# ServiceFoundation/partisan

Hardware: AMD Instinct MI355X
Metric: simulated node-rounds/sec (+ msgs/sec), 1M-node HyParView+Plumtree (higher is better)
Workload: dtype u32

## Files before the change

### partisan_amd/csrc/psim_engine.hip

```cpp
#include <hip/hip_runtime.h>
#include <rccl/rccl.h>

#include <algorithm>
#include <chrono>
#include <cstdio>
#include <cstdlib>
#include <cstring>
#include <new>
#include <set>
#include <vector>

#include "psim_comm.h"
#include "psim_device.h"
#include "psim_kernels.h"
#include "psim_wave.h"

using namespace psim;

namespace {

constexpr int BLK = 256;
constexpr uint32_t PREP_BLK = 1024;
#ifndef PSIM_PREP_NPT
#define PSIM_PREP_NPT 4
// ... 430 lines not shown
            nr++;
        });
    if (nr > FILL_REG) s_spill = 1;
    __syncthreads();
    const bool spill = s_spill != 0;
    bool over = false;
    for (uint32_t j = threadIdx.x; j < nb; j += blockDim.x) {
        const uint32_t c = hcnt[j];
        const uint32_t b0 = c ? atomicAdd(&gcnt[j], c) : 0u;
        over |= b0 + c > capb;
        hcnt[j] = j * capb + b0;
    }
    if (over) ctl[2] = 1;
    __syncthreads();
    const uint32_t wmask = (1u << wshift) - 1;
    auto put = [&](uint32_t g, uint32_t d, uint32_t cls) {
        const uint32_t j = d >> wshift, q = atomicAdd(&hcnt[j], 1u);
        if (q < (j + 1) * capb) pairs[q] = make_uint2((d & wmask) | (cls << 16), g);
    };
    if (!spill) {
#pragma unroll
        for (uint32_t k = 0; k < FILL_REG; k++)
            if (k < nr) put(rg[k], rk[k] & KEY_DST_MASK, rk[k] >> KEY_DST_BITS);
    } else {
        for (uint32_t step = blockIdx.x; step < nsteps; step += gridDim.x) route_step<DENSE>(in, step, spre, sbase, put);
    }
}

template <bool WRITE>
__global__ void __launch_bounds__(RB_STEP) k_owner_part(RouteIn in, uint32_t nsteps, uint32_t spb, uint32_t G,
                                                        uint32_t per, uint32_t* hist,
                                                        const uint32_t* __restrict__ off, Wire* __restrict__ out,
                                                        unsigned long long* mark, uint32_t capH, uint32_t capT,
                                                        const uint32_t* ctl, StatsIn st) {
    if (*ctl) return;
    if (mark && blockIdx.x == 0 && threadIdx.x == 0) *mark = __builtin_amdgcn_s_memrealtime();
    __shared__ uint32_t spre[RB_WAVES][65];
    __shared__ uint64_t sbase[RB_WAVES][64];
    if (!WRITE && blockIdx.x < st.nt) stats_tile(st, blockIdx.x, sbase);
    __shared__ uint32_t wc[RB_WAVES][64], wl[RB_WAVES][64];
    __shared__ uint32_t run[64], runl[64];
    __shared__ uint32_t tb[64];
    const uint32_t w = threadIdx.x >> 6, l = threadIdx.x & 63, nblk = gridDim.x;
    if (threadIdx.x < 64) {
        const uint32_t o = threadIdx.x;
        const bool q = WRITE && o < G;
        if (capH) {
            const uint32_t xs = XHDR + capH;
            run[o] = q ? o * xs + XHDR + off[o * nblk + blockIdx.x] - off[o * nblk] : 0u;
            runl[o] = q ? G * xs + o * capT + off[(G + o) * nblk + blockIdx.x] - off[(G + o) * nblk] : 0u;
            tb[o] = q ? G * xs + o * capT : 0u;
        } else {
            run[o] = q ? off[o * nblk + blockIdx.x] : 0u;
            runl[o] = q ? off[(G + o) * nblk + blockIdx.x] : 0u;
            tb[o] = q ? off[(G + o) * nblk] : 0u;
        }
    }
    if (!WRITE && blockIdx.x == 0 && threadIdx.x == 0) hist[2 * G * nblk] = 0;
    const uint32_t s_end = min(nsteps, (blockIdx.x + 1) * spb);
    for (uint32_t step = blockIdx.x * spb; step < s_end; step++) {
        const uint32_t i = step * RB_STEP + threadIdx.x;
        const uint32_t c = i < in.n_src ? in.ocnt[i] : 0u;
        uint32_t inc = c;
        for (int o = 1; o < 64; o <<= 1) {
            const uint32_t y = __shfl_up(inc, o);
            if (l >= (uint32_t)o) inc += y;
        }
        __syncthreads();
        spre[w][l + 1] = inc;
        if (l == 0) spre[w][0] = 0;
        sbase[w][l] = i < in.n_src ? in.obase[i] : 0ull;
        const uint32_t T = __shfl(inc, 63);
        __syncthreads();
        const uint32_t* pre = spre[w];
        auto rec_at = [&](uint32_t t, uint64_t& g) -> uint32_t {
            if (t >= T) return 0xFFFFFFFFu;
            uint32_t a = 0, b = 64;
            while (b - a > 1) {
                const uint32_t mid = (a + b) >> 1;
                if (pre[mid] <= t) a = mid; else b = mid;
            }
            g = sbase[w][a] + (t - pre[a]);
            return (in.okey[g] & KEY_DST_MASK) / per;
        };
        uint32_t cnt = 0, cntl = 0;
        for (uint32_t t0 = 0; t0 < T; t0 += 64) {
            uint64_t g = 0;
            const uint32_t o = rec_at(t0 + l, g);
            const bool lg = o != 0xFFFFFFFFu && wire_long(in.rec[g].tt);
            for (uint64_t todo = __ballot(o != 0xFFFFFFFFu); todo;) {
                const uint32_t q = __builtin_amdgcn_readlane(o, __ffsll((long long)todo) - 1);
                const uint64_t m = __ballot(o == q), ml = __ballot(o == q && lg);
                cnt += l == q ? (uint32_t)__popcll(m) : 0u;
                cntl += l == q ? (uint32_t)__popcll(ml) : 0u;
                todo &= ~m;
            }
        }
        wc[w][l] = cnt;
        wl[w][l] = cntl;
        __syncthreads();
        if (WRITE) {
            uint32_t B = 0, BL = 0;
            if (l < G) {
                B = run[l];
                BL = runl[l];
                for (uint32_t v = 0; v < w; v++) { B += wc[v][l]; BL += wl[v][l]; }
            }
            for (uint32_t t0 = 0; t0 < T; t0 += 64) {
                uint64_t g = 0;
                const uint32_t o = rec_at(t0 + l, g);
                uint4 x0 = make_uint4(0, 0, 0, 0), x1 = x0, x2 = x0, x3 = x0;
                if (o != 0xFFFFFFFFu) {
                    const uint4* sp = reinterpret_cast<const uint4*>(&in.rec[g]);
                    x0 = sp[0]; x1 = sp[1]; x2 = sp[2]; x3 = sp[3];
                }
                const bool lg = o != 0xFFFFFFFFu && wire_long(x0.z);
                uint32_t pos = 0, lpos = 0;
                for (uint64_t todo = __ballot(o != 0xFFFFFFFFu); todo;) {
                    const uint32_t q = __builtin_amdgcn_readlane(o, __ffsll((long long)todo) - 1);
                    const uint64_t m = __ballot(o == q), ml = __ballot(o == q && lg);
                    const uint64_t below = (1ull << l) - 1ull;
                    if (o == q) {
                        pos = __builtin_amdgcn_readlane(B, q) + (uint32_t)__popcll(m & below);
                        lpos = __builtin_amdgcn_readlane(BL, q) + (uint32_t)__popcll(ml & below);
                    }
                    B += l == q ? (uint32_t)__popcll(m) : 0u;
                    BL += l == q ? (uint32_t)__popcll(ml) : 0u;
                    todo &= ~m;
                }
                if (o != 0xFFFFFFFFu) {
                    if (lg) {
                        x1.w = lpos - tb[o];
                        if (!capH || x1.w < capT) {
                            out[lpos].q[0] = x2;
                            out[lpos].q[1] = x3;
                        }
                    }
                    if (!capH || pos < (o + 1) * (XHDR + capH)) {
                        out[pos].q[0] = x0;
                        out[pos].q[1] = x1;
                    }
                }
            }
        }
        __syncthreads();
        if (threadIdx.x < G)
            for (uint32_t v = 0; v < RB_WAVES; v++) { run[threadIdx.x] += wc[v][threadIdx.x]; runl[threadIdx.x] += wl[v][threadIdx.x]; }
    }
    if (!WRITE) {
        __syncthreads();
        if (threadIdx.x < G) {
            hist[threadIdx.x * nblk + blockIdx.x] = run[threadIdx.x];
            hist[(G + threadIdx.x) * nblk + blockIdx.x] = runl[threadIdx.x];
        }
    }
}

constexpr uint32_t OO_THREADS = 1024;
__global__ void k_owner_offsets(const uint32_t* hoff, uint32_t nblk, uint32_t G, uint64_t* d_off, uint64_t* cnt,
                                uint64_t* xw, uint32_t capH, uint32_t capT, uint32_t* ctl, uint32_t round,
                                uint32_t rank, Wire* sendbuf, StatsIn st) {
    __shared__ uint32_t smh, smt;
    __shared__ uint64_t ssum[64];
    __shared__ uint64_t sred[OO_THREADS / 64][64];
    const uint32_t q = threadIdx.x;
    const bool dead = *ctl != 0;
    if (capH) {
        const uint32_t xs = XHDR + capH;
        uint32_t mh = 0, mt = 0;
        for (uint32_t o = 0; o < G && !dead; o++) {
            mh = max(mh, hoff[(o + 1) * nblk] - hoff[o * nblk]);
            mt = max(mt, hoff[(G + o + 1) * nblk] - hoff[(G + o) * nblk]);
        }
        const bool over = !dead && (mh > capH || mt > capT);
        {
            const uint32_t c = q & 63, g = q >> 6, ng = OO_THREADS / 64;
            uint64_t v = 0;
            if (c < NST) {
#pragma unroll 4
                for (uint32_t b = g; b < st.nt; b += ng) v += st.tiles[(size_t)b * NST + c];
            }
            sred[g][c] = v;
            __syncthreads();
            if (g == 0) {
                uint64_t u = 0;
                for (uint32_t k = 0; k < ng; k++) u += sred[k][c];
                ssum[c] = u;
            }
        }
        __syncthreads();
        for (uint32_t o = 0; o < G; o++) {
            uint64_t* hw = reinterpret_cast<uint64_t*>(sendbuf + (size_t)o * xs);
            const uint64_t c = dead ? 0ull
                                    : (uint64_t)(hoff[(o + 1) * nblk] - hoff[o * nblk]) |
                                          ((uint64_t)(hoff[(G + o + 1) * nblk] - hoff[(G + o) * nblk]) << 32);
            if (q == 0) { hw[XH_CNT] = c; hw[XH_ABORT] = dead || over ? 1u : 0u; hw[XH_MH] = mh; hw[XH_MT] = mt; }
            if (q < NST) hw[XH_STATS + q] = ssum[q];
            if (q == 1) st.hout[PIN_XCNT + o] = c;
        }
        if (q == 0) {
            st.hout[NST] = st.out[NST];
            st.hout[NST + 1] = st.out[NST + 1];
            if (st.outx_top) st.hout0[PIN_OUTX] = *st.outx_top;
            if (over) { ctl[1] = round; __threadfence(); ctl[0] = 3; }
        }
        return;
    }
    if (q <= 2 * G) d_off[q] = hoff[q * nblk];
    if (cnt && q < G)
        cnt[q] = dead ? 0ull
                      : (uint64_t)(hoff[(q + 1) * nblk] - hoff[q * nblk]) |
                            ((uint64_t)(hoff[(G + q + 1) * nblk] - hoff[(G + q) * nblk]) << 32);
    if (!xw) return;
    if (q == 0) {
        uint32_t mh = 0, mt = 0;
        for (uint32_t o = 0; o < G && !dead; o++) {
            mh = max(mh, hoff[(o + 1) * nblk] - hoff[o * nblk]);
            mt = max(mt, hoff[(G + o + 1) * nblk] - hoff[(G + o) * nblk]);
        }
        xw[1] = mh;
        xw[2] = mt;
        smh = mh; smt = mt;
        if (capH && !dead && (mh > capH || mt > capT)) { ctl[1] = round; __threadfence(); ctl[0] = 3; }
    }
    __syncthreads();
    if (q < 128) xw[3 + q] = q == rank ? smh : q == 64 + rank ? smt : 0u;
}




__device__ __forceinline__ void block_sort_lds(uint32_t* sv, uint32_t* p, uint32_t k) {
    uint32_t P = 1;
    while (P < k) P <<= 1;
    for (uint32_t t = threadIdx.x; t < P; t += blockDim.x) sv[t] = t < k ? p[t] : 0xFFFFFFFFu;
    __syncthreads();
    for (uint32_t kk = 2; kk <= P; kk <<= 1) {
        for (uint32_t jj = kk >> 1; jj > 0; jj >>= 1) {
            for (uint32_t t = threadIdx.x; t < P; t += blockDim.x) {
                const uint32_t u = t ^ jj;
                if (u > t) {
                    const uint32_t a = sv[t], b = sv[u];
                    if ((a > b) == ((t & kk) == 0)) { sv[t] = b; sv[u] = a; }
                }
            }
            __syncthreads();
        }
    }
    for (uint32_t t = threadIdx.x; t < k; t += blockDim.x) p[t] = sv[t];
    __syncthreads();
}

__device__ __forceinline__ void sort_run_block(uint32_t* p, uint32_t k, uint32_t* y, uint32_t* sv) {
    for (uint32_t c0 = 0; c0 < k; c0 += RUN_LDS) block_sort_lds(sv, p + c0, min(RUN_LDS, k - c0));
    uint32_t* x = p;
    for (uint32_t wd = RUN_LDS; wd < k; wd *= 2) {
        for (uint32_t a0 = threadIdx.x * 2 * wd; a0 < k; a0 += blockDim.x * 2 * wd) {
            const uint32_t m0 = min(a0 + wd, k), e0 = min(a0 + 2 * wd, k);
            uint32_t u = a0, v = m0, o = a0;
            while (u < m0 && v < e0) y[o++] = x[u] <= x[v] ? x[u++] : x[v++];
            while (u < m0) y[o++] = x[u++];
            while (v < e0) y[o++] = x[v++];
        }
        __syncthreads();
        uint32_t* z = x; x = y; y = z;
    }
    if (x != p)
        for (uint32_t t = threadIdx.x; t < k; t += blockDim.x) p[t] = x[t];
    __syncthreads();
}

__device__ __forceinline__ void wave_sort64(uint32_t* p, uint32_t k) {
    const uint32_t l = threadIdx.x & 63;
    uint32_t v = l < k ? p[l] : 0xFFFFFFFFu;
#pragma unroll
    for (uint32_t kk = 2; kk <= 64; kk <<= 1) {
#pragma unroll
        for (uint32_t j = kk >> 1; j > 0; j >>= 1) {
            const uint32_t u = (uint32_t)__shfl_xor((int)v, (int)j);
            const bool keep_min = ((l & j) == 0) == ((l & kk) == 0);
            v = keep_min ? min(v, u) : max(v, u);
        }
    }
    if (l < k) p[l] = v;
}

__device__ __forceinline__ uint4 wire_piece(const Wire* __restrict__ heads, const Wire* __restrict__ tails,
                                            uint32_t k, uint32_t p) {
    if (p == 0) return heads[k].q[0];
    const uint32_t tt = heads[k].q[0].z;
    const uint4 h1 = heads[k].q[1];
    const bool lng = wire_long(tt);
    if (p == 1) return make_uint4(h1.x, h1.y, h1.z, lng ? 0u : h1.w);
    return lng ? tails[h1.w].q[p - 2] : make_uint4(0, 0, 0, 0);
}

__device__ __forceinline__ uint4 rec_piece(const Msg* __restrict__ rec, uint32_t k, uint32_t p) {
    const uint4 v = reinterpret_cast<const uint4*>(&rec[k])[p];
    if (!PSIM_SHORT_TAIL) return v;
    const uint32_t tt = (uint32_t)__builtin_amdgcn_update_dpp(0, (int)v.z, 0x00, 0xF, 0xF, false);
    return p < 2 || wire_long(tt) ? v : make_uint4(0, 0, 0, 0);
}

template <bool WIRE>
__global__ void __launch_bounds__(RR_THREADS) k_bucket_route(
    uint32_t n, uint32_t wshift, uint32_t regcap, const uint32_t* __restrict__ base,
    const uint2* __restrict__ pairs, const Msg* __restrict__ rec, const Wire* __restrict__ heads,
    const Wire* __restrict__ tails, uint32_t* rank, unsigned long long* cb,
    unsigned long long* bmask, uint32_t* in_beg, uint32_t* idx, uint32_t* tmp, Msg* __restrict__ inbox, uint64_t* hm,
    uint64_t cap, uint32_t* ctl, const uint32_t* gcnt, uint32_t capb, uint32_t round1, StatsIn st, uint32_t lcap) {
    if (*ctl) return;
    extern __shared__ __attribute__((aligned(16))) uint32_t sm[];
    __shared__ __attribute__((aligned(16))) uint32_t spart[RR_THREADS + 4];
    uint32_t& s_nl = spart[RR_THREADS];
    const uint32_t W = 1u << wshift, wmask = W - 1, b = blockIdx.x;
    uint32_t* cnt = sm;
    uint32_t* bs = sm + W;
    unsigned long long* mk = reinterpret_cast<unsigned long long*>(sm + 2 * W);
    uint32_t* pre = bs;
    uint32_t s0, s1, q0;
    if (gcnt) {
        if (b == 0) stats_final(st, reinterpret_cast<uint64_t(*)[64]>(sm));
        const uint32_t nb = gridDim.x, per_t = (nb + blockDim.x - 1) / blockDim.x;
        const uint32_t t0 = min(nb, threadIdx.x * per_t), t1 = min(nb, t0 + per_t);
        uint32_t v = 0;
        for (uint32_t j = t0; j < t1; j++) v += gcnt[j];
        uint32_t m;
        const uint32_t run = block_excl<uint32_t, RR_THREADS>(v, &m);
        if (b >= t0 && b < t1) {
            uint32_t x = run;
            for (uint32_t j = t0; j < b; j++) x += gcnt[j];
            spart[RR_THREADS + 1] = x;
        }
        __syncthreads();
        s0 = spart[RR_THREADS + 1];
        s1 = s0 + gcnt[b];
        q0 = b * capb;
        if (ctl[2] || m > cap) {
            if (b == 0 && threadIdx.x == 0) {
                *(hm + (PIN_OVF - PIN_M)) = max(m, 1u);
                if (round1) { ctl[1] = round1 - 1; __threadfence(); ctl[0] = 2; }
            }
            return;
        }
    } else {
        s0 = base[b]; s1 = base[b + 1]; q0 = s0;
        if (base[gridDim.x] > cap) return;
    }
    pairs += q0;
    rank += q0;
    uint32_t* const ix = lcap && s1 - s0 <= lcap ? sm + 4 * W : idx + s0;
    for (uint32_t j = threadIdx.x; j < 4 * W; j += blockDim.x) sm[j] = 0;
    if (threadIdx.x == 0) s_nl = 0;
    __syncthreads();
    auto count = [&](const uint2& x) {
        const uint32_t dl = x.x & wmask, cls = x.x >> 16;
        const uint32_t r = atomicAdd(&cnt[dl], 1u);
        if (cls == KEY_BCAST) {
            atomicAdd(&bs[dl], 1u);
            const uint32_t a0 = WIRE ? heads[x.y].q[1].x : rec[x.y].a0;
            atomicOr(&mk[dl], 1ull << (a0 % PSIM_MSG_SLOTS));
        } else if (cls) {
            atomicAdd(&bs[dl], cls);
        }
        return r;
    };
    const uint32_t np = s1 - s0;
    const bool inreg = np <= regcap * blockDim.x;
    uint2 px[RR_REG];
    uint32_t pr[RR_REG];
    if (inreg) {
#pragma unroll
        for (uint32_t k = 0; k < RR_REG; k++) {
            const uint32_t p = threadIdx.x + k * blockDim.x;
            px[k] = p < np ? pairs[p] : make_uint2(0, 0);
        }
#pragma unroll
        for (uint32_t k = 0; k < RR_REG; k++)
            if (threadIdx.x + k * blockDim.x < np) pr[k] = count(px[k]);
    } else {
        for (uint32_t p = threadIdx.x; p < np; p += blockDim.x) rank[p] = count(pairs[p]);
    }
    __syncthreads();
    const uint32_t per = W / RR_THREADS, j0 = threadIdx.x * per;
    uint32_t sum = 0;
    for (uint32_t j = 0; j < per; j++) sum += cnt[j0 + j];
    {
        uint32_t tot;
        spart[threadIdx.x] = block_excl<uint32_t, RR_THREADS>(sum, &tot) + sum;
    }
    for (uint32_t dl = threadIdx.x; dl < W; dl += blockDim.x) {
        const uint32_t d = (b << wshift) + dl;
        if (d >= n) break;
        cb[d] = cnt[dl] | ((unsigned long long)bs[dl] << 32);
        bmask[d] = mk[dl];
    }
    __syncthreads();
    uint32_t run = spart[threadIdx.x] - sum;
    for (uint32_t j = 0; j < per; j++) {
        pre[j0 + j] = run;
        run += cnt[j0 + j];
    }
    __syncthreads();
    for (uint32_t dl = threadIdx.x; dl < W; dl += blockDim.x) {
        const uint32_t d = (b << wshift) + dl;
        if (d >= n) break;
        in_beg[d] = s0 + pre[dl];
    }
    if (b == gridDim.x - 1 && threadIdx.x == 0) {
        in_beg[n] = s1;
        *hm = s1;
        if (s1 > hm[PIN_MMAX - PIN_M]) hm[PIN_MMAX - PIN_M] = s1;
    }
    if (inreg) {
#pragma unroll
        for (uint32_t k = 0; k < RR_REG; k++)
            if (threadIdx.x + k * blockDim.x < np) ix[pre[px[k].x & wmask] + pr[k]] = px[k].y;
    } else {
        for (uint32_t p = threadIdx.x; p < np; p += blockDim.x) {
            const uint2 x = pairs[p];
            ix[pre[x.x & wmask] + rank[p]] = x.y;
        }
    }
    __syncthreads();
    uint32_t* sv = reinterpret_cast<uint32_t*>(mk);
    uint32_t* ll = sv + RUN_LDS;
    for (uint32_t dl = threadIdx.x; dl < W; dl += blockDim.x) {
        const uint32_t k = cnt[dl];
        if (k < 2) continue;
        if (k > RUN_SHORT) {
            ll[atomicAdd(&s_nl, 1u)] = dl;
            continue;
        }
        uint32_t* q = ix + pre[dl];
        uint32_t v[RUN_SHORT];
#pragma unroll
        for (uint32_t t = 0; t < RUN_SHORT; t++) v[t] = t < k ? q[t] : 0xFFFFFFFFu;
#pragma unroll
        for (uint32_t r = 0; r < RUN_SHORT; r++) {
#pragma unroll
            for (uint32_t t = r & 1; t + 1 < RUN_SHORT; t += 2) {
                const uint32_t lo_ = v[t], hi_ = v[t + 1];
                v[t] = min(lo_, hi_);
                v[t + 1] = max(lo_, hi_);
            }
        }
#pragma unroll
        for (uint32_t t = 0; t < RUN_SHORT; t++)
            if (t < k) q[t] = v[t];
    }
    __syncthreads();
    const uint32_t nl = s_nl, wv = threadIdx.x >> 6, nwv = blockDim.x >> 6;
    for (uint32_t q = wv; q < nl; q += nwv) {
        const uint32_t dl = ll[q], k = cnt[dl];
        if (k <= 64) wave_sort64(ix + pre[dl], k);
    }
    __syncthreads();
    for (uint32_t q = 0; q < nl; q++) {
        const uint32_t dl = ll[q], k = cnt[dl];
        if (k > 64) sort_run_block(ix + pre[dl], k, tmp + s0 + pre[dl], sv);
    }
    __syncthreads();
    const uint32_t m4 = (s1 - s0) * 4, bd = blockDim.x;
    for (uint32_t t = threadIdx.x; t < m4; t += 2 * bd) {
        const uint32_t t2 = t + bd;
        uint4 a, c = make_uint4(0, 0, 0, 0);
        if (WIRE) {
            a = wire_piece(heads, tails, ix[t >> 2], t & 3);
            if (t2 < m4) c = wire_piece(heads, tails, ix[t2 >> 2], t2 & 3);
        } else {
            a = rec_piece(rec, ix[t >> 2], t & 3);
            if (t2 < m4) c = rec_piece(rec, ix[t2 >> 2], t2 & 3);
        }
        reinterpret_cast<uint4*>(&inbox[s0 + (t >> 2)])[t & 3] = a;
        if (t2 < m4) reinterpret_cast<uint4*>(&inbox[s0 + (t2 >> 2)])[t2 & 3] = c;
    }
}

constexpr uint64_t NODE_STATE_BYTES = 416;

__device__ __forceinline__ bool due(uint32_t period, uint32_t r, uint32_t start) {
    return period > 0 && r > start && ((r - start) % period) == 0;
}

#ifdef PSIM_BOUND_TERMS
enum { BT_RESP, BT_TIMER, BT_PUSH, BT_PUSH_NE, BT_NPUSH, BT_LAZY, BT_ON, BT_NL, BT_LC, BT_CRASH, BT_XBOT,
       BT_BUMP, BT_TOTAL, BT_C, BT_QUIET, BT_ROUNDS, BT_N };
__device__ unsigned long long g_bterm[BT_N];
#define BTERM(k, v) (bt[k] += (v))
#else
#define BTERM(k, v) ((void)0)
#endif

__global__ void __launch_bounds__(BLK) k_node_prep(RoundArgs a, const unsigned long long* bmask, uint64_t* packed,
                                                   uint64_t* part, uint32_t* ocnt, unsigned long long* btot,
                                                   uint32_t per, uint64_t* tiles, uint32_t* gcnt, uint32_t ngcnt) {
    if (*a.ctl) return;
    for (uint32_t j = blockIdx.x * blockDim.x + threadIdx.x; j < ngcnt; j += gridDim.x * blockDim.x) gcnt[j] = 0;
    if (gcnt && blockIdx.x == 0 && threadIdx.x == 0) const_cast<uint32_t*>(a.ctl)[2] = 0;
    __shared__ unsigned long long s_up, s_drop, s_b, s_w, s_qp, s_qf;
    if (threadIdx.x == 0) { s_up = 0; s_drop = 0; s_b = 0; s_w = 0; s_qp = 0; s_qf = 0; }
    if (blockIdx.x == 0 && threadIdx.x == 0) {
        a.ktime[0] = ~0ull; a.ktime[1] = 0; *a.n_slow = 0; *a.n_pt = 0;
        if (a.n_shuf) *a.n_shuf = 0;
        if (a.n_lite) { a.n_lite[0] = 0; a.n_lite[1] = 0; a.n_lite[2] = 0; a.n_lite[3] = 0; }
        if (a.n_ptl) { a.n_ptl[0] = 0; a.n_ptl[1] = 0; a.n_ptl[2] = 0; a.n_ptl[3] = 0; }
        if (a.n_stop) *a.n_stop = 0;
    }
    __syncthreads();
    if (a.upart && a.upart_dirty)
        for (uint32_t g = blockIdx.x * blockDim.x + threadIdx.x; g < a.n_nodes; g += gridDim.x * blockDim.x)
            a.upart[g] = (a.flags[g] & F_UP) ? (upart_t)a.part[g] : UPART_DOWN;
    unsigned long long up = 0, drop = 0, bs = 0, ws = 0;
    unsigned long long qp = 0, qf = 0;
#ifdef PSIM_BOUND_TERMS
    unsigned long long bt[BT_N] = {};
#endif
    const uint32_t i0 = blockIdx.x * per, i1 = min(a.n_local, i0 + per);
    struct PrepIn {
        uint8_t f;
        unsigned long long cbi;
        uint32_t st, org;
        unsigned long long bm;
    };
    auto prep_in = [&](uint32_t i) {
        PrepIn q{0, 0ull, 0u, 0u, 0ull};
        if (i < i1) {
            q.f = a.flags[a.lo + i];
            q.cbi = a.in_cb[i];
            q.st = a.start[i];
            q.org = a.pl ? 0u : a.origin[i];
            q.bm = a.pl ? 0ull : bmask[i];
        }
        return q;
    };
    auto node = [&](uint32_t i, const PrepIn& cur) -> uint64_t {
        uint8_t f = cur.f;
        uint64_t b = 0;
        uint32_t w = 0;
        const unsigned long long cbi = cur.cbi;
        uint32_t c = (uint32_t)cbi;
        const uint32_t st_ = cur.st;
        const uint32_t org_ = cur.org;
        const unsigned long long bm_ = cur.bm;
        if (f & F_UP) {
            uint32_t st = st_, r = a.round;
            if (a.pl) {
                const Hdr& x = a.hdr[i];
                bool pending = x.join_contact != PSIM_NONE;
                bool per = due(a.periodic, r, st);
                bool leave = x.pad1[0] != 0;
                if (a.strategy == PSIM_STRATEGY_FULL)
                    b = a.fanout ? (uint64_t)c + a.fanout + 1
                                 : ((uint64_t)c + 2 + (leave ? 1 : 0)) * (a.n_nodes + 1);
                else
                {
                    const uint64_t vn = x.act_n, vg = vn + c + 1;
                    b = (uint64_t)c + (pending ? 1 + 2 * vg : 0) + (per ? 1 + vg : 0) + (leave ? vn : 0) + 1;
                }
                w = c > 0 || (pending && !x.have) || per || leave;
            } else {
                bool origin = org_ != 0;
                const Hdr& x = a.hdr[i];
                const bool promo = a.random_promotion && due(a.promotion_period, r, st);
                b = (cbi >> 32) + (st == r && x.join_contact != PSIM_NONE ? 1u : 0u) + (promo ? 1u : 0u) +
                    (due(a.shuffle_period, r, st) ? 1u : 0u);
                BTERM(BT_RESP, cbi >> 32);
                BTERM(BT_TIMER, b - (cbi >> 32));
                const unsigned long long bm = c ? bm_ : 0ull;
                const uint32_t pushes = (uint32_t)__popcll(bm) + (origin ? 1u : 0u);
                const bool lazy = a.plumtree && due(a.lazy_tick_period, r, st);
                uint32_t lazy_add = 0, push_sum = 0, union_sum = 0;
                if (pushes) {
                    const uint4 r0 = *reinterpret_cast<const uint4*>(a.pt_rt + (size_t)i * RT_WORDS);
                    const uint2 cn = *reinterpret_cast<const uint2*>(a.pt_rt + (size_t)i * RT_WORDS + RT_EN);
                    const uint32_t rts[4] = {r0.x, r0.y, r0.z, r0.w};
                    auto push = [&](uint32_t root) {
                        uint32_t ne = PSIM_PT_MEMBERS_CAP, nl = 0, ne0 = 0;
#pragma unroll
                        for (int k = 0; k < PSIM_PT_ROOTS; k++)
                            if (rts[k] == root) {
                                ne0 = (cn.x >> (8 * k)) & 0xFFu;
                                ne = max(ne, ne0);
                                nl = (cn.y >> (8 * k)) & 0xFFu;
                            }
                        const uint32_t pb = min(2u * PSIM_ACTIVE_CAP, ne + c);
                        push_sum += pb;
                        lazy_add += nl + c;
                        union_sum += min(pb + nl + c, max((uint32_t)PSIM_PT_MEMBERS_CAP, ne0 + nl) + c);
                        BTERM(BT_PUSH, min(2u * PSIM_ACTIVE_CAP, ne + c));
                        BTERM(BT_PUSH_NE, min(2u * PSIM_ACTIVE_CAP, ne));
                        BTERM(BT_NPUSH, 1);
                        BTERM(BT_NL, nl);
                        BTERM(BT_LC, c);
                    };
                    for (unsigned long long m = bm; m; m &= m - 1) push(a.slots[PSIM_MSG_SLOTS + __ffsll(m) - 1]);
                    if (origin) push((a.lo + i) | PSIM_MAP_BIT);
                }
                if (lazy) {
                    const uint32_t fo = (uint32_t)f >> F_OUTN_SHIFT;
                    const uint32_t on = fo < 15 ? fo : (uint32_t)x.out_n;
                    const uint32_t pl = min(push_sum + min((uint32_t)PSIM_PT_OUT_CAP, on + lazy_add), on + union_sum);
                    b += pl;
                    BTERM(BT_LAZY, pl - push_sum);
                    BTERM(BT_ON, on);
                } else {
                    b += push_sum;
                }
                if (pushes) BTERM(BT_C, c);
                bool exits = false;
                if (a.crash_round) {
                    const uint4* ar = reinterpret_cast<const uint4*>(a.act + (size_t)i * PSIM_ACTIVE_CAP);
                    const uint4 a0 = ar[0], a1 = ar[1];
                    const uint32_t av[8] = {a0.x, a0.y, a0.z, a0.w, a1.x, a1.y, a1.z, a1.w};
                    uint32_t cv[PSIM_CONN_CAP] = {};
                    const uint32_t cn = x.conn_n;
                    if (cn) {
                        const uint4* cr = reinterpret_cast<const uint4*>(a.conn + (size_t)i * PSIM_CONN_CAP);
                        const uint4 c0 = cr[0], c1 = cr[1];
                        cv[0] = c0.x; cv[1] = c0.y; cv[2] = c0.z; cv[3] = c0.w;
                        cv[4] = c1.x; cv[5] = c1.y; cv[6] = c1.z; cv[7] = c1.w;
                    }
#pragma unroll
                    for (int k = 0; k < PSIM_ACTIVE_CAP; k++)
                        if ((uint32_t)k < x.act_n && av[k] < a.n_nodes && av[k] != a.lo + i &&
                            crashed_now(a, av[k])) {
                            b++;
                            BTERM(BT_CRASH, 1);
                            bool down = false;
#pragma unroll
                            for (int j = 0; j < PSIM_CONN_CAP; j++) down |= (uint32_t)j < cn && cv[j] == (av[k] | PSIM_CONN_DOWN);
                            exits |= !down;
                        }
#pragma unroll
                    for (int j = 0; j < PSIM_CONN_CAP; j++)
                        exits |= (uint32_t)j < cn && !(cv[j] & PSIM_CONN_DOWN) && crashed_now(a, cv[j] & KEY_DST_MASK);
                }
                const uint32_t fon = (uint32_t)f >> F_OUTN_SHIFT;
                const bool quiet_ok = a.lazy_tick_period == 1 && !a.lazy_wake && !(f & F_LAZY);
                w = c > 0 || st == r || exits || (fon && !quiet_ok) || origin ||
                    (a.random_promotion && (f & F_LOWACT) && due(a.promotion_period, r, st)) ||
                    due(a.shuffle_period, r, st);
                if (a.xbot) {
                    const bool xb = due(a.xbot_period, r, st);
                    const uint32_t cl = x.conn_cl;
                    b += (xb ? 2u : 0u) + cl;
                    BTERM(BT_XBOT, (xb ? 2u : 0u) + cl);
                    w = w || xb || cl;
                }
                if (w && b == 0) { b = 1; BTERM(BT_BUMP, 1); }
                if (!w && fon && lazy) {
                    qp++;
                    qf += fon < 15 ? fon : (uint32_t)x.out_n;
                    BTERM(BT_QUIET, 1);
                    b = 0;
                }
            }
            up++;
        } else {
            drop += c;
        }
        bs += b;
        ws += w;
        BTERM(BT_TOTAL, b);
        return (b << 32) | w;
    };
    PrepIn q[PREP_CHUNK], qn[PREP_CHUNK];
    const uint32_t cstep = PREP_CHUNK * blockDim.x;
#pragma unroll
    for (uint32_t k = 0; k < PREP_CHUNK; k++) q[k] = prep_in(i0 + threadIdx.x + k * blockDim.x);
    for (uint32_t c0 = i0 + threadIdx.x; c0 < i1; c0 += cstep) {
        uint64_t pk[PREP_CHUNK];
#pragma unroll
        for (uint32_t k = 0; k < PREP_CHUNK; k++) {
            const uint32_t i = c0 + k * blockDim.x;
            pk[k] = i < i1 ? node(i, q[k]) : 0ull;
        }
#pragma unroll
        for (uint32_t k = 0; k < PREP_CHUNK; k++) qn[k] = prep_in(c0 + cstep + k * blockDim.x);
#pragma unroll
        for (uint32_t k = 0; k < PREP_CHUNK; k++) {
            const uint32_t i = c0 + k * blockDim.x;
            if (i < i1) {
                packed[i] = pk[k];
                ocnt[i] = 0;
            }
        }
#pragma unroll
        for (uint32_t k = 0; k < PREP_CHUNK; k++) q[k] = qn[k];
    }
#ifdef PSIM_BOUND_TERMS
    if (blockIdx.x == 0 && threadIdx.x == 0) bt[BT_ROUNDS] = 1;
    for (int k = 0; k < BT_N; k++) {
        unsigned long long v = bt[k];
        for (int o = 32; o > 0; o >>= 1) v += __shfl_xor(v, o);
        if ((threadIdx.x & 63) == 0 && v) atomicAdd(&g_bterm[k], v);
    }
#endif
    for (int o = 32; o > 0; o >>= 1) {
        up += __shfl_xor(up, o);
        drop += __shfl_xor(drop, o);
        bs += __shfl_xor(bs, o);
        ws += __shfl_xor(ws, o);
        qp += __shfl_xor(qp, o);
        qf += __shfl_xor(qf, o);
    }
    if ((threadIdx.x & 63) == 0) {
        if (up) atomicAdd(&s_up, up);
        if (drop) atomicAdd(&s_drop, drop);
        if (bs) atomicAdd(&s_b, bs);
        if (ws) atomicAdd(&s_w, ws);
        if (qp) atomicAdd(&s_qp, qp);
        if (qf) atomicAdd(&s_qf, qf);
    }
    __syncthreads();
    if (threadIdx.x == 0) {
        tiles[blockIdx.x] = (s_b << 32) + s_w;
        if (blockIdx.x == gridDim.x - 1) tiles[gridDim.x] = 0;
    }
    if (threadIdx.x == 0) btot[blockIdx.x] = s_b;
    if (threadIdx.x < NST) {
        uint64_t v = threadIdx.x == ST_UP ? s_up : threadIdx.x == ST_DROPPED ? s_drop : threadIdx.x == ST_PROC ? s_qp
                   : threadIdx.x == ST_FAIL ? s_qf : threadIdx.x == ST_BYTES && !a.pl ? s_w * (2 * NODE_STATE_BYTES)
                   : 0ull;
        part[(size_t)blockIdx.x * NST + threadIdx.x] = v;
    }
}

struct DescIn {
    uint32_t in_beg, cnt, start, origin;
};
__device__ __forceinline__ DescIn desc_in(const RoundArgs& a, uint32_t li, uint64_t pk,
                                          const uint32_t* __restrict__ in_beg,
                                          const unsigned long long* __restrict__ cb,
                                          const uint32_t* __restrict__ start) {
    DescIn d{0, 0, 0, 0};
    if (pk & 1u) {
        d.in_beg = in_beg[li];
        d.cnt = (uint32_t)cb[li];
        d.start = start[li];
        d.origin = a.plumtree && !a.pl ? a.origin[li] : 0u;
    }
    return d;
}

__device__ __forceinline__ void desc_entry(const RoundArgs& a, uint32_t li, uint64_t P, uint64_t pk, const DescIn& d,
                                           uint4* __restrict__ desc, uint64_t* __restrict__ obase, uint32_t* nact,
                                           unsigned long long tot, uint64_t* hout, uint64_t cap, uint32_t* ctl) {
    obase[li] = P >> 32;
    if (li == a.n_local) {
        *nact = (uint32_t)P;
        obase[li] = tot;
        hout[PIN_TOTAL] = tot;
        if (tot > hout[PIN_TMAX]) hout[PIN_TMAX] = tot;
        if (cap && tot + 1 > cap) { ctl[1] = a.round; __threadfence(); ctl[0] = 1; }
        return;
    }
    if (!(pk & 1u)) return;
    if (d.cnt > DESC_CNT_MASK) hout[PIN_BIGIN] = 1;
    const uint32_t st = d.start, r = a.round;
    const uint32_t tf = (a.random_promotion && due(a.promotion_period, r, st) ? DESC_PROMO : 0u) |
                        (due(a.shuffle_period, r, st) ? DESC_SHUFFLE : 0u) |
                        (a.plumtree && due(a.lazy_tick_period, r, st) ? DESC_LAZY : 0u) |
                        (d.origin ? DESC_ORIGIN : 0u);
    const uint32_t xb = a.xbot && due(a.xbot_period, r, st) ? DESC_XBOT_BIT : 0u;
    desc[(uint32_t)P] = make_uint4(a.lo + li, d.in_beg, d.cnt | xb | (tf << 28), (uint32_t)(P >> 32));
}

__device__ unsigned long long btot_sum(const unsigned long long* btot, uint32_t nbt) {
    __shared__ unsigned long long s_w[PREP_BLK / 64], s_tot;
    unsigned long long t = 0;
    for (uint32_t j = threadIdx.x; j < nbt; j += blockDim.x) t += btot[j];
    for (int o = 32; o > 0; o >>= 1) t += __shfl_xor(t, o);
    if ((threadIdx.x & 63) == 0) s_w[threadIdx.x >> 6] = t;
    __syncthreads();
    if (threadIdx.x == 0) {
        unsigned long long u = 0;
        for (uint32_t k = 0; k < blockDim.x / 64; k++) u += s_w[k];
        s_tot = u;
    }
    __syncthreads();
    return s_tot;
}


__global__ void __launch_bounds__(PREP_BLK) k_desc(const uint64_t* __restrict__ packed,
                                                  const uint64_t* __restrict__ tiles, uint32_t per,
                                                  const uint32_t* __restrict__ in_beg,
                                                  const unsigned long long* __restrict__ cb,
                                                  const uint32_t* __restrict__ start, RoundArgs a,
                                                  uint4* __restrict__ desc, uint64_t* __restrict__ obase,
                                                  uint32_t* nact, const unsigned long long* btot,
                                                  uint32_t nranges, uint64_t* hout, uint64_t cap, uint32_t* ctl) {
    if (*ctl) return;
    const bool last = blockIdx.x == gridDim.x - 1;
    const uint32_t r0 = blockIdx.x * DESC_RANGES;
    const uint32_t i0 = r0 * per, i1 = min(a.n_local, i0 + DESC_RANGES * per);
    uint64_t tp = 0;
#pragma unroll
    for (uint32_t k = 0; k < DESC_RANGES; k++) {
        const uint32_t j = threadIdx.x + k * PREP_BLK;
        tp += j < r0 ? tiles[j] : 0ull;
    }
    uint32_t li = i0 + threadIdx.x;
    uint64_t pk = li < i1 ? packed[li] : 0ull;
    DescIn d = desc_in(a, li, pk, in_beg, cb, start);
    const unsigned long long tot = last ? btot_sum(btot, nranges) : 0ull;
    uint64_t carry;
    (void)block_excl<uint64_t, PREP_BLK>(tp, &carry);
    for (uint32_t k = i0; k < i1; k += PREP_BLK) {
        if (k != i0) {
            li = k + threadIdx.x;
            pk = li < i1 ? packed[li] : 0ull;
            d = desc_in(a, li, pk, in_beg, cb, start);
        }
        uint64_t pass;
        const uint64_t e = block_excl<uint64_t, PREP_BLK>(pk, &pass);
        if (li < i1) desc_entry(a, li, carry + e, pk, d, desc, obase, nact, 0ull, hout, cap, ctl);
        carry += pass;
    }
    if (last && threadIdx.x == 0)
        desc_entry(a, a.n_local, carry, 0ull, DescIn{0, 0, 0, 0}, desc, obase, nact, tot, hout, cap, ctl);
}

enum { H_AIN = 0, H_PIN = 1, H_AOUT = 2, H_PFILL = 3, H_HOP = 4, H_NUP = 5 * PSIM_HIST_BINS,
       H_DELIV, H_LAST, H_LINKS, H_N };

__device__ __forceinline__ uint32_t hbin(uint32_t v) { return v < PSIM_HIST_BINS ? v : PSIM_HIST_BINS - 1; }

__global__ void k_hist_out(const Hdr* __restrict__ hdr, const uint32_t* __restrict__ act,
                           const uint32_t* __restrict__ pas, const uint8_t* __restrict__ flags, uint32_t lo,
                           uint32_t n, uint64_t tbit, uint32_t* indeg_a, uint32_t* indeg_p,
                           unsigned long long* hist) {
    __shared__ unsigned long long sh[H_N];
    for (uint32_t j = threadIdx.x; j < H_N; j += blockDim.x) sh[j] = 0;
    __syncthreads();
    const uint32_t i = blockIdx.x * blockDim.x + threadIdx.x;
    if (i < n && (flags[lo + i] & F_UP)) {
        const Hdr& x = hdr[i];
        const uint32_t me = lo + i;
        uint32_t out = 0;
        for (uint32_t k = 0; k < x.act_n; k++) {
            const uint32_t p = act[(size_t)i * PSIM_ACTIVE_CAP + k];
            if (p == me) continue;
            out++;
            if (flags[p] & F_UP) { atomicAdd(&indeg_a[p], 1u); atomicAdd(&sh[H_LINKS], 1ull); }
        }
        for (uint32_t k = 0; k < x.pas_n; k++) {
            const uint32_t p = pas[(size_t)i * PSIM_PASSIVE_CAP + k];
            if (p != me && (flags[p] & F_UP)) atomicAdd(&indeg_p[p], 1u);
        }
        atomicAdd(&sh[H_AOUT * PSIM_HIST_BINS + hbin(out)], 1ull);
        atomicAdd(&sh[H_PFILL * PSIM_HIST_BINS + hbin(x.pas_n)], 1ull);
        atomicAdd(&sh[H_NUP], 1ull);
        if (tbit && ((((uint64_t)x.aux << 32) | x.have) & tbit)) {
            atomicAdd(&sh[H_DELIV], 1ull);
            atomicAdd(&sh[H_HOP * PSIM_HIST_BINS + hbin(x.trk_hop)], 1ull);
            if (x.trk_round != PSIM_NONE) atomicMax(&sh[H_LAST], (unsigned long long)x.trk_round);
        }
    }
    __syncthreads();
    for (uint32_t j = threadIdx.x; j < H_N; j += blockDim.x) {
        if (!sh[j]) continue;
        if (j == H_LAST) atomicMax(&hist[j], sh[j]);
        else atomicAdd(&hist[j], sh[j]);
    }
}

__global__ void k_hist_in(const uint32_t* __restrict__ indeg_a, const uint32_t* __restrict__ indeg_p,
                          const uint8_t* __restrict__ flags, uint32_t lo, uint32_t n, unsigned long long* hist) {
    __shared__ unsigned long long sh[2 * PSIM_HIST_BINS];
    for (uint32_t j = threadIdx.x; j < 2 * PSIM_HIST_BINS; j += blockDim.x) sh[j] = 0;
    __syncthreads();
    const uint32_t i = blockIdx.x * blockDim.x + threadIdx.x;
    if (i < n && (flags[lo + i] & F_UP)) {
        atomicAdd(&sh[hbin(indeg_a[lo + i])], 1ull);
        atomicAdd(&sh[PSIM_HIST_BINS + hbin(indeg_p[lo + i])], 1ull);
    }
    __syncthreads();
    for (uint32_t j = threadIdx.x; j < 2 * PSIM_HIST_BINS; j += blockDim.x)
        if (sh[j]) atomicAdd(&hist[H_AIN * PSIM_HIST_BINS + j], sh[j]);
}

__global__ void k_pack_act(const Hdr* __restrict__ hdr, const uint32_t* __restrict__ act, uint32_t n,
                           uint32_t* gact, uint8_t* gan) {
    const uint32_t i = blockIdx.x * blockDim.x + threadIdx.x;
    if (i >= n) return;
    const uint32_t k = hdr[i].act_n;
    gan[i] = (uint8_t)k;
    for (uint32_t j = 0; j < PSIM_ACTIVE_CAP; j++) gact[(size_t)i * PSIM_ACTIVE_CAP + j] = act[(size_t)i * PSIM_ACTIVE_CAP + j];
}

__global__ void k_hist_sym(const uint8_t* __restrict__ gan, const uint32_t* __restrict__ act,
                           const uint8_t* __restrict__ flags, uint32_t n, unsigned long long* sym) {
    const uint32_t i = blockIdx.x * blockDim.x + threadIdx.x;
    if (i >= n || !(flags[i] & F_UP)) return;
    uint32_t c = 0;
    for (uint32_t k = 0; k < gan[i]; k++) {
        const uint32_t p = act[(size_t)i * PSIM_ACTIVE_CAP + k];
        if (p == i || p >= n || !(flags[p] & F_UP)) continue;
        for (uint32_t q = 0; q < gan[p]; q++)
            if (act[(size_t)p * PSIM_ACTIVE_CAP + q] == i) { c++; break; }
    }
    if (c) atomicAdd(sym, (unsigned long long)c);
}

__global__ void k_cc_init(const uint8_t* __restrict__ flags, uint32_t n, uint32_t* L) {
    const uint32_t i = blockIdx.x * blockDim.x + threadIdx.x;
    if (i < n) L[i] = (flags[i] & F_UP) ? i : PSIM_NONE;
}

__global__ void k_cc_hook(const uint32_t* __restrict__ off, const uint8_t* __restrict__ gan,
                          const uint32_t* __restrict__ act, const uint8_t* __restrict__ flags, uint32_t n,
                          uint32_t* L, uint32_t* changed) {
    const uint32_t i = blockIdx.x * blockDim.x + threadIdx.x;
    if (i >= n || !(flags[i] & F_UP)) return;
    const uint32_t* row = act + (off ? (size_t)off[i] : (size_t)i * PSIM_ACTIVE_CAP);
    for (uint32_t k = 0; k < gan[i]; k++) {
        const uint32_t p = row[k];
        if (p == i || p >= n || !(flags[p] & F_UP)) continue;
        const uint32_t a = L[i], b = L[p];
        if (a < b) { if (atomicMin(&L[p], a) > a) *changed = 1; }
        else if (b < a) { if (atomicMin(&L[i], b) > b) *changed = 1; }
    }
}

__global__ void k_cc_jump(uint32_t n, uint32_t* L) {
    const uint32_t i = blockIdx.x * blockDim.x + threadIdx.x;
    if (i >= n || L[i] == PSIM_NONE) return;
    uint32_t r = L[i];
    while (L[r] != r) r = L[r];
    L[i] = r;
}

__global__ void k_cc_count(const uint32_t* __restrict__ L, uint32_t n, uint32_t* size, unsigned long long* comps) {
    const uint32_t i = blockIdx.x * blockDim.x + threadIdx.x;
    if (i >= n || L[i] == PSIM_NONE) return;
    atomicAdd(&size[L[i]], 1u);
    if (L[i] == i) atomicAdd(comps, 1ull);
}

__global__ void k_cc_max(const uint32_t* __restrict__ size, uint32_t n, unsigned long long* largest) {
    const uint32_t i = blockIdx.x * blockDim.x + threadIdx.x;
    if (i < n && size[i]) atomicMax(largest, (unsigned long long)size[i]);
}

enum { SL_VFILL = 0, SL_IFILL = 1, SL_OUT = 2, SL_NUP = 3 * PSIM_HIST_BINS, SL_VSUM, SL_ISUM, SL_DANG, SL_SELF,
       SL_DUP, SL_IVL, SL_IVC, SL_VMAX, SL_N };
enum { SG_LINKS = PSIM_HIST_BINS, SG_MUTUAL, SG_INMAX, SG_ISOL, SG_COMPS, SG_LARGEST, SG_N };
enum { SF_NUP = 0, SF_MIN, SF_MAX, SF_SUM, SF_AGREE, SF_N };
constexpr uint32_t SH_NPB = BLK;

DEV void sh_row_load(const uint32_t* __restrict__ row, uint32_t n, uint32_t& a, uint32_t& b) {
    const uint32_t l = lane_id();
    a = l < n ? row[l] : PSIM_NONE;
    b = n > 64 && 64 + l < n ? row[64 + l] : PSIM_NONE;
}
DEV void sh_row_first(uint32_t a, uint32_t b, uint32_t n, bool& fa, bool& fb) {
    const uint32_t l = lane_id();
    fa = l < n; fb = 64 + l < n;
    for (uint32_t j = 0; j + 1 < n; j++) {
        const uint32_t v = j < 64 ? shfl(a, (int)j) : shfl(b, (int)(j - 64));
        if (l > j && a == v) fa = false;
        if (64 + l > j && b == v) fb = false;
    }
}
DEV uint32_t sh_wave_sum(uint32_t v) {
    for (int d = 32; d; d >>= 1) v += (uint32_t)__shfl_xor((int)v, d);
    return v;
}
DEV bool sh_live(const uint8_t* __restrict__ flags, uint32_t N, uint32_t id) {
    return id < N && (flags[id] & F_UP);
}

__global__ void __launch_bounds__(BLK) k_sh_rows(const Hdr* __restrict__ hdr, const uint32_t* __restrict__ sview,
                                                 const uint8_t* __restrict__ flags, uint32_t lo, uint32_t n,
                                                 uint32_t N, uint32_t v2, uint8_t* cnt,
                                                 const uint32_t* __restrict__ off, uint32_t* adj,
                                                 unsigned long long* sl) {
    __shared__ unsigned long long sh[SL_N];
    for (uint32_t j = threadIdx.x; j < SL_N; j += blockDim.x) sh[j] = 0;
    __syncthreads();
    const uint32_t l = lane_id();
    const uint32_t base = blockIdx.x * SH_NPB + (threadIdx.x >> 6) * 64;
    const uint32_t mine = base + l;
    uint32_t vn = 0, in_n = 0, o = 0, my_cnt = 0;
    if (mine < n && (flags[lo + mine] & F_UP)) {
        vn = min((uint32_t)hdr[mine].act_n, (uint32_t)PSIM_SVIEW_CAP);
        in_n = hdr[mine].pas_n;
        if (off) o = off[lo + mine];
    }
    const uint64_t up = ballot(mine < n && (flags[lo + mine] & F_UP));
    uint64_t todo = off ? ballot(vn != 0) : up;
    unsigned long long s_vsum = 0, s_isum = 0, s_dang = 0, s_self = 0, s_dup = 0, s_vmax = 0;
    while (todo) {
        const int k = ffs64(todo);
        todo &= todo - 1;
        const uint32_t i = base + (uint32_t)k, me = lo + i;
        const uint32_t len = shfl(vn, k);
        uint32_t a, b;
        bool fa, fb;
        sh_row_load(sview + (size_t)i * PSIM_SVIEW_CAP, len, a, b);
        sh_row_first(a, b, len, fa, fb);
        const uint64_t oa = ballot(fa && a != me), ob = ballot(fb && b != me);
        const uint64_t la = ballot(fa && a != me && sh_live(flags, N, a));
        const uint64_t lb = ballot(fb && b != me && sh_live(flags, N, b));
        if (off) {
            const uint32_t at = shfl(o, k);
            if ((la >> l) & 1) adj[at + popc(la & lt_mask())] = a;
            if ((lb >> l) & 1) adj[at + popc(la) + popc(lb & lt_mask())] = b;
            continue;
        }
        const uint32_t links = popc(la) + popc(lb), others = popc(oa) + popc(ob);
        const uint32_t distinct = popc(ballot(fa)) + popc(ballot(fb));
        if (l == (uint32_t)k) my_cnt = links;
        s_vsum += len; s_dang += others - links; s_self += distinct - others; s_dup += len - distinct;
        s_vmax = len > s_vmax ? len : s_vmax;
        const uint32_t inn = v2 ? shfl(in_n, k) : 0;
        s_isum += inn;
        if (l == 0) {
            atomicAdd(&sh[SL_VFILL * PSIM_HIST_BINS + hbin(len)], 1ull);
            atomicAdd(&sh[SL_OUT * PSIM_HIST_BINS + hbin(others)], 1ull);
            if (v2) atomicAdd(&sh[SL_IFILL * PSIM_HIST_BINS + hbin(inn)], 1ull);
        }
    }
    if (off) return;
    if (mine < n) cnt[lo + mine] = (uint8_t)my_cnt;
    if (l == 0) {
        atomicAdd(&sh[SL_NUP], (unsigned long long)popc(up));
        atomicAdd(&sh[SL_VSUM], s_vsum); atomicAdd(&sh[SL_ISUM], s_isum); atomicAdd(&sh[SL_DANG], s_dang);
        atomicAdd(&sh[SL_SELF], s_self); atomicAdd(&sh[SL_DUP], s_dup); atomicMax(&sh[SL_VMAX], s_vmax);
    }
    __syncthreads();
    for (uint32_t j = threadIdx.x; j < SL_N; j += blockDim.x) {
        if (!sh[j]) continue;
        if (j == SL_VMAX) atomicMax(&sl[j], sh[j]);
        else atomicAdd(&sl[j], sh[j]);
    }
}

DEV bool sh_has(const uint32_t* __restrict__ off, const uint8_t* __restrict__ cnt, const uint32_t* __restrict__ adj,
                uint32_t p, uint32_t id) {
    const uint32_t* row = adj + off[p];
    for (uint32_t q = 0, c = cnt[p]; q < c; q++)
        if (row[q] == id) return true;
    return false;
}

__global__ void __launch_bounds__(BLK) k_sh_inv(const Hdr* __restrict__ hdr, const uint32_t* __restrict__ sinv,
                                                const uint8_t* __restrict__ flags, uint32_t lo, uint32_t n,
                                                uint32_t N, const uint32_t* __restrict__ off,
                                                const uint8_t* __restrict__ cnt, const uint32_t* __restrict__ adj,
                                                unsigned long long* sl) {
    const uint32_t l = lane_id();
    const uint32_t base = blockIdx.x * SH_NPB + (threadIdx.x >> 6) * 64;
    const uint32_t mine = base + l;
    uint32_t in_n = 0;
    if (mine < n && (flags[lo + mine] & F_UP)) in_n = min((uint32_t)hdr[mine].pas_n, (uint32_t)PSIM_SVIEW_CAP);
    uint64_t todo = ballot(in_n != 0);
    uint32_t ivl = 0, ivc = 0;
    while (todo) {
        const int k = ffs64(todo);
        todo &= todo - 1;
        const uint32_t i = base + (uint32_t)k, me = lo + i;
        const uint32_t len = shfl(in_n, k);
        uint32_t a, b;
        bool fa, fb;
        sh_row_load(sinv + (size_t)i * PSIM_SVIEW_CAP, len, a, b);
        sh_row_first(a, b, len, fa, fb);
        if (fa && a != me && sh_live(flags, N, a)) { ivl++; ivc += sh_has(off, cnt, adj, a, me) ? 1u : 0u; }
        if (fb && b != me && sh_live(flags, N, b)) { ivl++; ivc += sh_has(off, cnt, adj, b, me) ? 1u : 0u; }
    }
    ivl = sh_wave_sum(ivl); ivc = sh_wave_sum(ivc);
    if (l == 0 && ivl) atomicAdd(&sl[SL_IVL], (unsigned long long)ivl);
    if (l == 0 && ivc) atomicAdd(&sl[SL_IVC], (unsigned long long)ivc);
}

__global__ void k_sh_rank_tot(const uint32_t* __restrict__ E, uint32_t per, uint32_t W, uint32_t npad,
                              uint32_t* base, unsigned long long* tot) {
    if (blockIdx.x || threadIdx.x) return;
    unsigned long long mx = 0;
    for (uint32_t r = 0; r < W; r++) {
        const uint32_t b = E[min(npad, r * per)], e = E[min(npad, (r + 1) * per)];
        base[r] = b;
        mx = max(mx, (unsigned long long)(e - b));
    }
    tot[0] = mx;
}
__global__ void k_sh_shift(uint32_t* E, uint32_t npad, uint32_t per, uint32_t slot,
                           const uint32_t* __restrict__ base) {
    const uint32_t i = blockIdx.x * blockDim.x + threadIdx.x;
    if (i >= npad) return;
    const uint32_t r = i / per;
    E[i] = E[i] - base[r] + r * slot;
}

__global__ void k_sh_links(const uint32_t* __restrict__ off, const uint8_t* __restrict__ cnt,
                           const uint32_t* __restrict__ adj, uint32_t n, uint32_t* indeg, unsigned long long* sg) {
    __shared__ unsigned long long sh[2];
    if (threadIdx.x < 2) sh[threadIdx.x] = 0;
    __syncthreads();
    const uint32_t i = blockIdx.x * blockDim.x + threadIdx.x;
    const uint32_t c = i < n ? cnt[i] : 0;
    if (c) {
        const uint32_t* row = adj + off[i];
        uint32_t m = 0;
        for (uint32_t k = 0; k < c; k++) {
            const uint32_t p = row[k];
            if (p >= n) continue;
            atomicAdd(&indeg[p], 1u);
            m += sh_has(off, cnt, adj, p, i) ? 1u : 0u;
        }
        atomicAdd(&sh[0], (unsigned long long)c);
        if (m) atomicAdd(&sh[1], (unsigned long long)m);
    }
    __syncthreads();
    if (threadIdx.x < 2 && sh[threadIdx.x]) atomicAdd(&sg[SG_LINKS + threadIdx.x], sh[threadIdx.x]);
}

__global__ void k_sh_in(const uint32_t* __restrict__ indeg, const uint8_t* __restrict__ cnt,
                        const uint8_t* __restrict__ flags, uint32_t n, unsigned long long* sg) {
    __shared__ unsigned long long sh[SG_ISOL + 1];
    for (uint32_t j = threadIdx.x; j <= SG_ISOL; j += blockDim.x) sh[j] = 0;
    __syncthreads();
    const uint32_t i = blockIdx.x * blockDim.x + threadIdx.x;
    if (i < n && (flags[i] & F_UP)) {
        const uint32_t d = indeg[i];
        atomicAdd(&sh[hbin(d)], 1ull);
        atomicMax(&sh[SG_INMAX], (unsigned long long)d);
        if (!d && !cnt[i]) atomicAdd(&sh[SG_ISOL], 1ull);
    }
    __syncthreads();
    for (uint32_t j = threadIdx.x; j <= SG_ISOL; j += blockDim.x) {
        if (!sh[j]) continue;
        if (j == SG_INMAX) atomicMax(&sg[j], sh[j]);
        else atomicAdd(&sg[j], sh[j]);
    }
}

__global__ void k_sh_low(const uint8_t* __restrict__ flags, uint32_t lo, uint32_t n, uint32_t* low) {
    const uint32_t i = blockIdx.x * blockDim.x + threadIdx.x;
    if (i < n && (flags[lo + i] & F_UP)) atomicMin(low, i);
}
__global__ void __launch_bounds__(BLK) k_sh_full(const uint32_t* __restrict__ fbits, const uint8_t* __restrict__ flags,
                                                 uint32_t lo, uint32_t n, uint32_t fw, uint32_t tomb,
                                                 const uint32_t* __restrict__ low, unsigned long long* sf) {
    const uint32_t i = blockIdx.x * (BLK / 64) + (threadIdx.x >> 6);
    if (i >= n || !(flags[lo + i] & F_UP)) return;
    const uint32_t* row = fbits + (size_t)i * 2 * fw;
    const uint32_t* ref = fbits + (size_t)*low * 2 * fw;
    uint32_t c = 0;
    bool differs = false;
    for (uint32_t w = lane_id(); w < fw; w += 64) {
        const uint32_t q = tomb ? row[w] & ~row[fw + w] : row[w];
        const uint32_t r = tomb ? ref[w] & ~ref[fw + w] : ref[w];
        c += (uint32_t)__popc(q);
        differs |= q != r;
    }
    c = sh_wave_sum(c);
    const bool agree = ballot(differs) == 0;
    if (lane_id() == 0) {
        atomicAdd(&sf[SF_NUP], 1ull);
        atomicMin(&sf[SF_MIN], (unsigned long long)c);
        atomicMax(&sf[SF_MAX], (unsigned long long)c);
        atomicAdd(&sf[SF_SUM], (unsigned long long)c);
        if (agree) atomicAdd(&sf[SF_AGREE], 1ull);
    }
}

template <typename T>
struct DBuf {
    T* p = nullptr;
    size_t n = 0;
    int ensure(size_t want, int headroom = 0) {
        if (want <= n) return PSIM_OK;
        static const bool trace = getenv("PSIM_TRACE_GROW") != nullptr;
        if (trace && want >= (1u << 20))
            std::fprintf(stderr, "psim: grow %zu -> %zu (want) x %zu B\n", n, want, sizeof(T));
        if (p) (void)hipFree(p);
        p = nullptr; n = 0;
        const size_t goal = want + want / 4 * (size_t)(headroom > 0 ? headroom : 0);
        size_t cap = 1024;
        while (cap < goal) cap <<= 1;
        if (headroom < 0) cap = want;
        if (cap * sizeof(T) > (1ull << 30)) {
            const size_t step = (64ull << 20) / sizeof(T);
            cap = (want + (headroom < 0 ? 0 : want / 8) + step - 1) / step * step;
        }
        if (hipMalloc(&p, cap * sizeof(T)) != hipSuccess) {
            size_t fr = 0, tot = 0;
            (void)hipGetLastError();
            if (hipMemGetInfo(&fr, &tot) == hipSuccess)
                std::fprintf(stderr, "psim: device allocation of %.2f GB failed (%.2f of %.2f GB free)\n",
                             cap * sizeof(T) / 1e9, fr / 1e9, tot / 1e9);
            p = nullptr;
            return PSIM_ENOMEM;
        }
        n = cap;
        return PSIM_OK;
    }
    int ensure_keep(size_t want, size_t keep, hipStream_t st) {
        if (want <= n) return PSIM_OK;
        if (!p || !keep) return ensure(want);
        DBuf<T> nb;
        TRY(nb.ensure(want));
        if (hipMemcpyAsync(nb.p, p, std::min(keep, n) * sizeof(T), hipMemcpyDeviceToDevice, st) != hipSuccess ||
            hipStreamSynchronize(st) != hipSuccess) {
            nb.release();
            return PSIM_EDEVICE;
        }
        release();
        p = nb.p; n = nb.n;
        return PSIM_OK;
    }
    int alloc(size_t want) {
        static const bool trace = getenv("PSIM_TRACE_GROW") != nullptr;
        if (trace && want >= (1u << 20)) std::fprintf(stderr, "psim: alloc %zu x %zu B\n", want, sizeof(T));
        if (hipMalloc(&p, std::max<size_t>(want, 1) * sizeof(T)) != hipSuccess) return PSIM_ENOMEM;
        n = want;
        if (hipMemset(p, 0, std::max<size_t>(want, 1) * sizeof(T)) != hipSuccess) return PSIM_EDEVICE;
        return PSIM_OK;
    }
    int alloc_on(size_t want, hipStream_t st) {
        if (hipMalloc(&p, std::max<size_t>(want, 1) * sizeof(T)) != hipSuccess) return PSIM_ENOMEM;
        n = want;
        if (hipMemsetAsync(p, 0, std::max<size_t>(want, 1) * sizeof(T), st) != hipSuccess) return PSIM_EDEVICE;
        return PSIM_OK;
    }
    void release() { if (p) (void)hipFree(p); p = nullptr; n = 0; }
};

template <typename T>
struct TmpBuf : DBuf<T> {
    TmpBuf() = default;
    TmpBuf(const TmpBuf&) = delete;
    TmpBuf& operator=(const TmpBuf&) = delete;
    ~TmpBuf() { this->release(); }
};

enum Kern { KT_EVENTS, KT_PREPARE, KT_CONSUME, KT_SCAN, KT_COMPACT, KT_SORT, KT_EXCHANGE, KT_GATHER,
            KT_STATS, KT_N };
const char* kKernName[KT_N] = {"events", "prepare", "consume", "scan", "compact", "sort",
                               "exchange", "gather", "stats"};

inline uint32_t grid_for(uint64_t n) { return (uint32_t)std::max<uint64_t>(1, (n + BLK - 1) / BLK); }

int bits_for(uint64_t n) {
    int b = 1;
    while (b < 32 && (1ull << b) < n) b++;
    return b;
}

constexpr uint64_t RESERVE_PER_NODE = 24;
constexpr uint64_t RCAP_PER_NODE = 4;
constexpr uint64_t RCAP_RESERVE = 8;
constexpr double RCAP_FREE_FRAC = 0.30;
constexpr double OUTBOX_SPARE = 0.12;

struct Shard {
    uint32_t idx = 0, lo = 0, n = 0;
    hipStream_t stream = nullptr;
    DBuf<uint8_t> flags, part;
    DBuf<upart_t> upart;
    DBuf<uint8_t> lite_cm;
    DBuf<uint32_t> crash_bits;
    DBuf<uint8_t> btab;
    DBuf<Hdr> hdr;
    DBuf<uint32_t> act, pas, pt_all, pt_com, pt_eag, pt_laz, pt_rt, start;
    DBuf<uint64_t> sentm, recvm, mapx;
    DBuf<uint32_t> mapx_top;
    DBuf<uint32_t> origin;
    DBuf<uint32_t> slots;
    DBuf<uint32_t> bc_roots, bc_msgs;
    DBuf<uint64_t> pt_out, outx;
    DBuf<uint32_t> conn;
    DBuf<uint32_t> outx_top;
    DBuf<uint32_t> ikeys, ivals;
    uint32_t m_in = 0;
    DBuf<Msg> outbox;
    DBuf<Wire> recvh, recvt;
    DBuf<uint32_t> wseg;
    std::vector<uint32_t> wseg_host;
    DBuf<Msg> inbox;
    DBuf<uint32_t> okey, ocnt, in_beg,
        d_nact, n_slow, n_pt, n_shuf, n_lite, n_ptl, rank, tmp, hist, hoff;
    DBuf<uint32_t> rtot, rbase;
    DBuf<uint32_t> gcnt;
    DBuf<unsigned long long> bmask;
    DBuf<uint2> pairs;
    DBuf<unsigned long long> cb;
    DBuf<unsigned long long> btot;
    DBuf<uint4> desc, desc_slow, desc_pt, desc_shuf, desc_lite, desc_ptl;
    DBuf<uint64_t> bound, pscan, obase, stat_part, stat_out, stat_tile, d_off;
    DBuf<uint8_t> cub_tmp;
    DBuf<uint32_t> ev_ids, ev_contacts, stop_ids, n_stop;
    bool tomb_live = false;
    DBuf<Wire> sendbuf;
    DBuf<uint32_t> sview, sinv, fbits, pay[2], pay_top;
    int pay_cur = 0;
    DBuf<uint8_t> faulted;
    DBuf<uint64_t> omit;
    std::vector<uint64_t> soff, scnt, lcnt;
    uint32_t pper = BLK;
    uint32_t pgrid = 0, cgrid = 0, rgrid = 0, tgrid = 0, sgrid = 0, lgrid = 0, qgrid = 0, egrid = 0;
    uint64_t* pin = nullptr;
    uint64_t* pin_dev = nullptr;
    static constexpr int MAXT = 32;
    hipEvent_t ev[MAXT][2];
    int tk[MAXT];
    int tn = 0;
    hipEvent_t wait_ev = nullptr;
    hipStream_t side[2] = {nullptr, nullptr};
    hipEvent_t fork_ev = nullptr, join_ev[2] = {nullptr, nullptr};
    bool ev_live = false;
    bool reserved = false;
    bool upart_valid = false;
    uint64_t rcap = 0;
    DBuf<uint32_t> ctl;
    uint64_t desc_cap = 0;
    uint32_t batch_round1 = 0;
    uint32_t stat_slot = 0;
    bool outx_short = false;
    uint32_t xcap_h = 0, xcap_t = 0;
    uint32_t xbatch = 1;
    uint64_t trace_tmax = 0, trace_mmax = 0;
};

}

struct psim_handle {
    psim_config cfg;
    uint32_t N = 0, G = 1, per = 0;
    int device = 0;
    uint32_t consume_blocks = 1024;
    uint32_t pt_blocks = 1024;
    uint32_t lite_blocks = 1024;
    psim::LiteKernel lite = {};
    uint32_t ptl_blocks = 1024;
    uint64_t round = 0;
    bool failed = false;
    std::vector<Shard*> shards;
    int rank = 0, world = 1;
    bool ranked = false;
    Comm* comm = nullptr;
    DBuf<uint64_t> comm_cnt;
    uint64_t x_records = 0, x_bytes = 0;
    std::vector<uint32_t> pend_crash, pend_join, pend_contact;
    std::vector<uint8_t> pend_join_mark;
    std::vector<uint32_t> pend_lv_a, pend_lv_t;
    std::vector<uint8_t> pend_part;
    bool pend_part_set = false, pend_part_clear = false;
    std::vector<uint32_t> pend_b_root, pend_b_msg;
    uint32_t slot_tab[2 * PSIM_MSG_SLOTS];
    uint32_t tracked_msg = PSIM_NONE;
    bool btab = false;
    uint32_t btab_hash = 0;
    uint32_t fw = 0;
    bool tomb = false;
    std::vector<uint8_t> started;
    std::set<uint64_t> nx_omit_s, nx_omit_r;
    std::vector<uint8_t> nx_faulted;
    size_t nx_nfaulted = 0;
    bool faults_dirty = false;
    uint32_t faults = 0, n_omit_s = 0, n_omit_r = 0;
    double kt_ms[KT_N] = {0};
    uint64_t kt_n[KT_N] = {0};
    bool phase_timers = false;
    uint32_t rb_blocks = RB_BLOCKS;
    uint32_t rr_reg = RR_REG;
    bool route_fused = true;
};

namespace {

inline bool local_route(const psim_handle* h) { return h->G == 1 && !h->ranked; }

constexpr int PTL_EARLY_DEFAULT = 0;
int ptl_early_knob() {
    static const int v = [] {
        const char* e = getenv("PSIM_PTL_EARLY");
        const int x = e && *e ? atoi(e) : -1;
        return x >= 0 && x <= 2 ? x : PTL_EARLY_DEFAULT;
    }();
    return v;
}

RoundArgs make_args(psim_handle* h, Shard* s) {
    RoundArgs a;
    memset(&a, 0, sizeof a);
    const psim_config& c = h->cfg;
    a.n_nodes = h->N; a.round = (uint32_t)h->round; a.seed = c.seed;
    a.lo = s->lo; a.n_local = s->n;
    a.max_active = c.max_active_size; a.min_active = c.min_active_size;
    a.max_passive = c.max_passive_size; a.arwl = c.arwl; a.prwl = c.prwl;
    a.k_active = c.k_active; a.k_passive = c.k_passive;
    a.shuffle_period = c.shuffle_period; a.promotion_period = c.promotion_period;
    a.random_promotion = c.random_promotion; a.plumtree = c.plumtree;
    a.lazy_tick_period = c.lazy_tick_period;
    a.tracked_msg = h->tracked_msg;
    a.origin = s->origin.p;
    a.slots = s->slots.p;
    a.flags = s->flags.p; a.part = s->part.p; a.hdr = s->hdr.p; a.crash_bits = s->crash_bits.p;
    a.upart = s->upart.p;
    a.lite_cm = s->lite_cm.p;
    a.btab = h->btab ? s->btab.p : nullptr;
    a.act = s->act.p; a.pas = s->pas.p; a.sentm = s->sentm.p; a.recvm = s->recvm.p;
    a.mapx = s->mapx.p; a.mapx_top = s->mapx_top.p;
    a.mapx_rows = (uint32_t)(s->mapx.n / IDMAP_EXT);
    a.pt_all = s->pt_all.p; a.pt_com = s->pt_com.p; a.pt_eag = s->pt_eag.p; a.pt_laz = s->pt_laz.p;
    a.pt_rt = s->pt_rt.p;
    a.pt_out = s->pt_out.p; a.outx = s->outx.p; a.outx_top = s->outx_top.p;
    a.conn = s->conn.p;
    a.outx_rows = (uint32_t)(s->outx.n / OUT_EXT);
    a.start = s->start.p;
    a.pl = c.manager == PSIM_MANAGER_PLUGGABLE;
    a.xbot = c.manager == PSIM_MANAGER_XBOT; a.xbot_period = c.xbot_period;
    a.ptl_split = ptl_early_knob() != 0;
    a.strategy = c.strategy; a.periodic = c.periodic_interval; a.scamp_c = c.scamp_c;
    a.fanout = c.fanout; a.fw = h->fw; a.tomb = h->tomb;
    a.fbits = s->fbits.p; a.sview = s->sview.p; a.sinv = s->sinv.p;
    a.ktime = reinterpret_cast<unsigned long long*>(s->stat_out.p + NST);
    a.ctl = s->ctl.p;
    a.desc_slow = s->desc_slow.p; a.n_slow = s->n_slow.p;
    a.desc_pt = s->desc_pt.p; a.n_pt = s->n_pt.p;
    a.desc_shuf = s->desc_shuf.p; a.n_shuf = s->n_shuf.p;
    a.desc_lite = s->desc_lite.p; a.n_lite = s->n_lite.p;
    a.desc_ptl = s->desc_ptl.p; a.n_ptl = s->n_ptl.p;
    a.stop_ids = s->stop_ids.p; a.n_stop = s->n_stop.p;
    a.faults = h->faults; a.n_omit_s = h->n_omit_s; a.n_omit_r = h->n_omit_r;
    a.faulted = s->faulted.p; a.omit = s->omit.p;
    return a;
}

int route_buffers(Shard* s, bool both_inboxes);

struct KTimer {
    Shard* s;
    int slot;
    KTimer(psim_handle* h, Shard* s_, int k) : s(s_), slot(-1) {
        if (!h->phase_timers || s->tn >= Shard::MAXT) return;
        slot = s->tn++;
        s->tk[slot] = k;
        (void)hipEventRecord(s->ev[slot][0], s->stream);
    }
    ~KTimer() {
        if (slot >= 0) (void)hipEventRecord(s->ev[slot][1], s->stream);
    }
};

void flush_timers(psim_handle* h, Shard* s) {
    for (int i = 0; i < s->tn; i++) {
        float ms = 0;
        if (hipEventElapsedTime(&ms, s->ev[i][0], s->ev[i][1]) != hipSuccess) continue;
        h->kt_ms[s->tk[i]] += ms;
        h->kt_n[s->tk[i]]++;
    }
    s->tn = 0;
}

constexpr uint32_t SCAN_ITEMS = 8, SCAN_TILE = BLK * SCAN_ITEMS;

template <typename T, uint32_t NT>
__device__ T block_excl(T v, T* total) {
    __shared__ T wsum[NT / 64];
    const uint32_t l = threadIdx.x & 63, wv = threadIdx.x >> 6;
    T x = v;
#pragma unroll
    for (int d = 1; d < 64; d <<= 1) {
        const T y = __shfl_up(x, d);
        if (l >= (uint32_t)d) x += y;
    }
    if (l == 63) wsum[wv] = x;
    __syncthreads();
    T base = 0, tot = 0;
#pragma unroll
    for (uint32_t k = 0; k < NT / 64; k++) {
        base += k < wv ? wsum[k] : T(0);
        tot += wsum[k];
    }
    __syncthreads();
    *total = tot;
    return base + x - v;
}

template <typename T, typename TI>
__global__ void __launch_bounds__(BLK) k_scan_tiles(const TI* __restrict__ in, uint32_t n, T* __restrict__ sums) {
    const size_t b0 = (size_t)blockIdx.x * SCAN_TILE + (size_t)threadIdx.x * SCAN_ITEMS;
    T v = 0;
#pragma unroll
    for (uint32_t k = 0; k < SCAN_ITEMS; k++) v += b0 + k < n ? in[b0 + k] : T(0);
    T tot;
    (void)block_excl(v, &tot);
    if (threadIdx.x == 0) sums[blockIdx.x] = tot;
}

constexpr uint32_t SUMS_LDS = 4096 + 2 * BLK;
template <typename T>
__global__ void __launch_bounds__(BLK) k_scan_sums(T* sums, uint32_t nt) {
    __shared__ T buf[SUMS_LDS];
    const bool lds = nt <= SUMS_LDS;
    T* p = lds ? buf : sums;
    if (lds) {
        for (uint32_t i = threadIdx.x; i < nt; i += BLK) buf[i] = sums[i];
        __syncthreads();
    }
    const uint32_t per = (nt + BLK - 1) / BLK, i0 = threadIdx.x * per, i1 = min(nt, i0 + per);
    T v = 0;
    for (uint32_t i = i0; i < i1; i++) v += p[i];
    T tot;
    T run = block_excl(v, &tot);
    for (uint32_t i = i0; i < i1; i++) {
        const T x = p[i];
        p[i] = run;
        run += x;
    }
    if (lds) {
        __syncthreads();
        for (uint32_t i = threadIdx.x; i < nt; i += BLK) sums[i] = buf[i];
    }
}

template <typename T, typename TI>
__global__ void __launch_bounds__(BLK) k_scan_apply(const TI* __restrict__ in, T* __restrict__ out, uint32_t n,
                                                   const T* __restrict__ sums) {
    const size_t b0 = (size_t)blockIdx.x * SCAN_TILE + (size_t)threadIdx.x * SCAN_ITEMS;
    T x[SCAN_ITEMS], v = 0;
#pragma unroll
    for (uint32_t k = 0; k < SCAN_ITEMS; k++) {
        x[k] = b0 + k < n ? in[b0 + k] : T(0);
        v += x[k];
    }
    T tot;
    T run = block_excl(v, &tot) + (sums ? sums[blockIdx.x] : T(0));
#pragma unroll
    for (uint32_t k = 0; k < SCAN_ITEMS; k++) {
        if (b0 + k < n) out[b0 + k] = run;
        run += x[k];
    }
}

template <typename T, typename TI>
int scan_excl(Shard* s, const TI* in, T* out, uint32_t n) {
    const uint32_t nt = (uint32_t)(((uint64_t)n + SCAN_TILE - 1) / SCAN_TILE);
    if (nt <= 1) {
        k_scan_apply<T, TI><<<1, BLK, 0, s->stream>>>(in, out, n, nullptr);
    } else {
        TRY(s->cub_tmp.ensure((size_t)nt * sizeof(T)));
        T* sums = reinterpret_cast<T*>(s->cub_tmp.p);
        k_scan_tiles<T, TI><<<nt, BLK, 0, s->stream>>>(in, n, sums);
        k_scan_sums<T><<<1, BLK, 0, s->stream>>>(sums, nt);
        k_scan_apply<T, TI><<<nt, BLK, 0, s->stream>>>(in, out, n, sums);
    }
    HIP_TRY(hipGetLastError());
    return PSIM_OK;
}

int scan_desc(Shard* s, const RoundArgs& a) {
    k_desc<<<(s->pgrid + DESC_RANGES - 1) / DESC_RANGES, PREP_BLK, 0, s->stream>>>(
        s->bound.p, s->pscan.p, s->pper, s->in_beg.p, s->cb.p, s->start.p, a, s->desc.p, s->obase.p, s->d_nact.p,
        s->btot.p, s->pgrid, s->pin_dev, s->desc_cap, s->ctl.p);
    HIP_TRY(hipGetLastError());
    return PSIM_OK;
}

int stream_wait(Shard* s) {
    HIP_TRY(hipEventRecord(s->wait_ev, s->stream));
    hipError_t e;
    while ((e = hipEventQuery(s->wait_ev)) == hipErrorNotReady) {
    }
    if (e != hipSuccess) {
        static bool said = false;
        if (!said) std::fprintf(stderr, "psim: event query: %s; synchronising\n", hipGetErrorString(e));
        said = true;
        HIP_TRY(hipStreamSynchronize(s->stream));
    }
    return PSIM_OK;
}

template <typename T>
T read1(Shard* s, const T* p) {
    T v{};
    (void)hipMemcpyAsync(&v, p, sizeof(T), hipMemcpyDeviceToHost, s->stream);
    (void)stream_wait(s);
    return v;
}

int upload(Shard* s, DBuf<uint32_t>& b, const std::vector<uint32_t>& v) {
    TRY(b.ensure(v.size()));
    HIP_TRY(hipMemcpyAsync(b.p, v.data(), v.size() * 4, hipMemcpyHostToDevice, s->stream));
    return PSIM_OK;
}

struct RoundCtl {
    bool crashes = false;
    uint64_t bcast_clear = 0;
};

int phase_events_prepare(psim_handle* h, Shard* s, const RoundCtl& ctl, RoundArgs& a, bool events = true,
                         bool batched = false, bool redo = false) {
    const uint32_t n = s->n;
    if (events && h->faults_dirty) {
        std::vector<uint64_t> keys(h->nx_omit_s.begin(), h->nx_omit_s.end());
        keys.insert(keys.end(), h->nx_omit_r.begin(), h->nx_omit_r.end());
        TRY(s->faulted.ensure(h->N));
        TRY(s->omit.ensure(std::max<size_t>(keys.size(), 1)));
        HIP_TRY(hipMemcpyAsync(s->faulted.p, h->nx_faulted.data(), h->N, hipMemcpyHostToDevice, s->stream));
        if (!keys.empty())
            HIP_TRY(hipMemcpyAsync(s->omit.p, keys.data(), keys.size() * 8, hipMemcpyHostToDevice, s->stream));
        HIP_TRY(hipStreamSynchronize(s->stream));
    }
    a = make_args(h, s);
    a.crash_round = ctl.crashes;
    a.upart_dirty = !s->upart_valid ||
                    (events && (ctl.crashes || !h->pend_join.empty() || h->pend_part_set || h->pend_part_clear));
    a.lazy_wake = !s->upart_valid || ((events || redo) && (h->pend_part_set || h->pend_part_clear ||
                                                            h->faults_dirty || !h->pend_lv_a.empty()));
    s->upart_valid = true;
    if (events) {
        KTimer t(h, s, KT_EVENTS);
        if (ctl.crashes) {
            TRY(upload(s, s->ev_ids, h->pend_crash));
            k_crash<<<grid_for(h->pend_crash.size()), BLK, 0, s->stream>>>(
                s->flags.p, s->crash_bits.p, s->ev_ids.p, (uint32_t)h->pend_crash.size());
        }
        if (!h->pend_join.empty()) {
            TRY(upload(s, s->ev_ids, h->pend_join));
            TRY(upload(s, s->ev_contacts, h->pend_contact));
            k_join<<<grid_for(h->pend_join.size()), BLK, 0, s->stream>>>(
                a, s->start.p, s->ev_ids.p, s->ev_contacts.p, (uint32_t)h->pend_join.size(),
                h->cfg.persist_epoch);
        }
        if (!h->pend_lv_a.empty()) {
            TRY(upload(s, s->ev_ids, h->pend_lv_a));
            TRY(upload(s, s->ev_contacts, h->pend_lv_t));
            k_leave_set<<<grid_for(h->pend_lv_a.size()), BLK, 0, s->stream>>>(
                s->hdr.p, s->lo, s->n, s->ev_ids.p, s->ev_contacts.p, (uint32_t)h->pend_lv_a.size());
        }
        if (h->pend_part_clear) HIP_TRY(hipMemsetAsync(s->part.p, 0, h->N, s->stream));
        if (h->pend_part_set)
            HIP_TRY(hipMemcpyAsync(s->part.p, h->pend_part.data(), h->N, hipMemcpyHostToDevice, s->stream));
        if (!h->pend_b_root.empty()) {
            const uint32_t k = (uint32_t)h->pend_b_root.size();
            k_bcast_reset<<<grid_for(n), BLK, 0, s->stream>>>(s->hdr.p, n, (uint32_t)ctl.bcast_clear,
                                                               (uint32_t)(ctl.bcast_clear >> 32));
            TRY(upload(s, s->bc_roots, h->pend_b_root));
            TRY(upload(s, s->bc_msgs, h->pend_b_msg));
            HIP_TRY(hipMemcpyAsync(s->slots.p, h->slot_tab, sizeof h->slot_tab, hipMemcpyHostToDevice, s->stream));
            k_origin<<<grid_for(k), BLK, 0, s->stream>>>(s->origin.p, s->lo, n, s->bc_roots.p, s->bc_msgs.p, k,
                                                          s->flags.p, false, s->ctl.p);
        }
    }
    {
        KTimer t(h, s, KT_PREPARE);
        a.in_cb = s->cb.p;
        {
            const uint32_t g = std::min<uint32_t>(std::max<uint32_t>(1, grid_for(n) / PREP_NPT), DESC_RANGES * PREP_BLK);
            s->pper = BLK * (uint32_t)(((uint64_t)n + (uint64_t)g * BLK - 1) / ((uint64_t)g * BLK));
            s->pgrid = std::max<uint32_t>(1, (uint32_t)(((uint64_t)n + s->pper - 1) / s->pper));
        }
        s->cgrid = std::min<uint32_t>(grid_for(n), h->consume_blocks);
        const bool hv = h->cfg.manager != PSIM_MANAGER_PLUGGABLE;
        s->rgrid = hv ? std::min<uint32_t>(grid_for(n), RELAY_MAX_BLOCKS) : 0;
        s->tgrid = hv && h->cfg.plumtree ? std::min<uint32_t>(grid_for(n), h->pt_blocks) : 0;
        s->sgrid = hv ? std::min<uint32_t>(grid_for(n), SHUF_MAX_BLOCKS) : 0;
        const uint32_t lnodes = h->lite.grid_nodes;
        s->lgrid = hv ? std::min<uint32_t>((uint32_t)((n + lnodes - 1) / lnodes), h->lite_blocks) : 0;
        const uint32_t qnodes = PTL_BLOCK;
        s->qgrid = hv && h->cfg.plumtree ? std::min<uint32_t>((uint32_t)((n + qnodes - 1) / qnodes), h->ptl_blocks) : 0;
        s->egrid = ptl_early_knob() ? s->qgrid : 0;
        TRY(s->stat_part.ensure((size_t)(s->pgrid + s->cgrid + s->rgrid + s->tgrid + s->sgrid + s->lgrid + s->qgrid + s->egrid) *
                                NST));
        k_node_prep<<<s->pgrid, BLK, 0, s->stream>>>(a, s->bmask.p, s->bound.p, s->stat_part.p, s->ocnt.p,
                                                     s->btot.p, s->pper, s->pscan.p, s->gcnt.p, (uint32_t)s->gcnt.n);
        TRY(scan_desc(s, a));
        if (batched) goto args;
        TRY(stream_wait(s));
        if (s->pin[PIN_BIGIN]) { s->pin[PIN_BIGIN] = 0; return PSIM_ENOMEM; }
        const uint64_t total = s->pin[PIN_TOTAL];
        if (total >= 0xFFFFFFFFull) return PSIM_ENOMEM;
        uint64_t want = total + 1;
        int headroom = 2;
        const char* rcap_init = getenv("PSIM_RCAP_INIT");
        if (local_route(h) && !s->rcap) {
            s->rcap = 4096;
            while (s->rcap < (uint64_t)n * RCAP_PER_NODE) s->rcap <<= 1;
            if (rcap_init) s->rcap = std::max<uint64_t>(16, strtoull(rcap_init, nullptr, 10));
        }
        if (!s->reserved) {
            s->reserved = true;
            size_t fr = 0, tot = 0;
            if (!getenv("PSIM_NO_RESERVE") && hipMemGetInfo(&fr, &tot) == hipSuccess) {
                const uint64_t per_rec = sizeof(Msg) + 3 * sizeof(uint32_t) + sizeof(uint2);
                const uint64_t per_slot = sizeof(Msg) + sizeof(uint32_t);
                uint64_t avail = fr + (uint64_t)s->outbox.n * sizeof(Msg) + (uint64_t)s->okey.n * 4;
                static const uint64_t res_pn = getenv("PSIM_RESERVE_PER_NODE")
                                                   ? strtoull(getenv("PSIM_RESERVE_PER_NODE"), nullptr, 10) : RESERVE_PER_NODE;
                static const uint64_t rcap_pn = getenv("PSIM_RCAP_RESERVE")
                                                    ? strtoull(getenv("PSIM_RCAP_RESERVE"), nullptr, 10) : RCAP_RESERVE;
                if (local_route(h) && !rcap_init) {
                    const uint64_t rc = (uint64_t)n * rcap_pn;
                    if (rc > s->rcap && (double)(rc * per_rec) <= RCAP_FREE_FRAC * (double)avail) s->rcap = rc;
                    const uint64_t held = s->rcap * per_rec;
                    avail = avail > held ? avail - held : 0;
                }
                const uint64_t r = std::min<uint64_t>((uint64_t)n * res_pn,
                                                      (uint64_t)((1.0 - OUTBOX_SPARE) * (double)avail) / per_slot);
                if (r > want) {
                    want = r;
                    headroom = -1;
                    s->outbox.release();
                    s->okey.release();
                }
            }
        } else if (want > s->outbox.n && s->outbox.n * sizeof(Msg) > (1ull << 30)) {
            std::fprintf(stderr, "psim: round %llu: outbox grows past its reservation (%zu -> %llu slots)\n",
                         (unsigned long long)h->round, s->outbox.n, (unsigned long long)want);
        }
        TRY(s->outbox.ensure(want, headroom));
        TRY(s->okey.ensure(want, headroom));
        if (local_route(h)) TRY(route_buffers(s, s->m_in == 0));
    }
args:
    a.in_beg = s->in_beg.p;
    a.desc = s->desc.p; a.n_alist = s->d_nact.p;
    a.rec_in = s->inbox.p;
    a.obase = s->obase.p;
    a.rec_out = s->outbox.p;
    a.okey = s->okey.p; a.ocnt = s->ocnt.p;
    a.stat_part = s->stat_part.p + (size_t)s->pgrid * NST;
    a.stat_relay = s->stat_part.p + (size_t)(s->pgrid + s->cgrid) * NST;
    a.stat_pt = s->stat_part.p + (size_t)(s->pgrid + s->cgrid + s->rgrid) * NST;
    a.stat_shuf = s->stat_part.p + (size_t)(s->pgrid + s->cgrid + s->rgrid + s->tgrid) * NST;
    a.stat_lite = s->stat_part.p + (size_t)(s->pgrid + s->cgrid + s->rgrid + s->tgrid + s->sgrid) * NST;
    a.stat_ptl = s->stat_part.p + (size_t)(s->pgrid + s->cgrid + s->rgrid + s->tgrid + s->sgrid + s->lgrid) * NST;
    a.stat_ptle = s->egrid ? a.stat_ptl + (size_t)s->qgrid * NST : nullptr;
    return PSIM_OK;
}

constexpr int PHASE_FUSED_DEFAULT = 3;

void launch_lite(psim_handle* h, Shard* s, const RoundArgs& a, hipStream_t st) {
    h->lite.kernel<<<s->lgrid, h->lite.block, 0, st>>>(a);
}

int phase_consume(psim_handle* h, Shard* s, RoundArgs& a) {
    if (a.pl && a.strategy == PSIM_STRATEGY_FULL) {
        uint64_t slots = (uint64_t)s->m_in + s->n + 1;
        if (slots > 0xFFFFFFFFull) return PSIM_ENOMEM;
        TRY(s->pay[s->pay_cur].ensure(slots * 2 * h->fw));
        if (h->tomb && !s->tomb_live) {
            DBuf<uint32_t>& in = s->pay[s->pay_cur ^ 1];
            const size_t rows = in.n / (2 * h->fw);
            if (rows)
                HIP_TRY(hipMemset2DAsync(in.p + h->fw, 2 * h->fw * 4, 0, h->fw * 4, rows, s->stream));
            s->tomb_live = true;
        }
        a.pay_out = s->pay[s->pay_cur].p;
        a.pay_in = s->pay[s->pay_cur ^ 1].p;
        a.pay_top = s->pay_top.p;
        a.pay_cap = (uint32_t)(s->pay[s->pay_cur].n / (2 * h->fw));
        HIP_TRY(hipMemsetAsync(s->pay_top.p, 0, 4, s->stream));
    }
    if (a.pl) {
        k_consume_pl<<<s->cgrid, BLK, 0, s->stream>>>(a);
    } else {
        k_relay<<<s->rgrid, BLK, 0, s->stream>>>(a);
        RoundArgs b = a;
        b.desc = s->desc_slow.p;
        b.n_alist = s->n_slow.p;
        static const bool conc_env = getenv("PSIM_CONCURRENT_PHASE") != nullptr;
        static const bool serial_env = getenv("PSIM_SERIAL_PHASE") != nullptr;
        const bool serial = serial_env || a.crash_round || !(conc_env || h->lite.side_by_side);
        static const int fused_env = [] {
            const char* e = getenv("PSIM_PHASE_FUSED");
            const int v = e && *e ? atoi(e) : PHASE_FUSED_DEFAULT;
            return v == 2 || v == 3 ? v : 0;
        }();
        const bool fused = fused_env && !a.crash_round && !serial_env && !conc_env && h->lite.kernel == k_lite_quarter;
        const int early = fused && fused_env == 3 && s->egrid ? ptl_early_knob() : 0;
        if (fused) {
            const uint32_t lg = fused_env == 3 ? s->lgrid : 0, eg = early == 1 ? s->egrid : 0;
            if (s->sgrid + s->cgrid + lg + eg)
                k_hv_phase<<<s->sgrid + s->cgrid + lg + eg, BLK, 0, s->stream>>>(a, s->sgrid, s->cgrid, eg);
            if (fused_env == 2) launch_lite(h, s, a, s->stream);
        } else if (serial) {
            k_shuf<<<s->sgrid, BLK, 0, s->stream>>>(a);
            launch_lite(h, s, a, s->stream);
            k_consume<<<s->cgrid, BLK, 0, s->stream>>>(b);
        } else {
            HIP_TRY(hipEventRecord(s->fork_ev, s->stream));
            HIP_TRY(hipStreamWaitEvent(s->side[0], s->fork_ev, 0));
            HIP_TRY(hipStreamWaitEvent(s->side[1], s->fork_ev, 0));
            k_consume<<<s->cgrid, BLK, 0, s->side[0]>>>(b);
            k_shuf<<<s->sgrid, BLK, 0, s->side[1]>>>(a);
            launch_lite(h, s, a, s->stream);
            for (int k = 0; k < 2; k++) {
                HIP_TRY(hipEventRecord(s->join_ev[k], s->side[k]));
                HIP_TRY(hipStreamWaitEvent(s->stream, s->join_ev[k], 0));
            }
        }
        if (s->qgrid) {
            if (early == 2) k_ptl_part<<<s->egrid, PTL_BLOCK, 0, s->stream>>>(a, PTL_EARLY);
            if (early) k_ptl_part<<<s->qgrid, PTL_BLOCK, 0, s->stream>>>(a, PTL_LATE);
            else k_ptl<<<s->qgrid, PTL_BLOCK, 0, s->stream>>>(a);
        }
        if (s->tgrid) {
            RoundArgs c = a;
            c.desc = s->desc_pt.p;
            c.n_alist = s->n_pt.p;
            c.stat_part = a.stat_pt;
            k_pt<<<s->tgrid, BLK, 0, s->stream>>>(c);
        }
    }
    HIP_TRY(hipGetLastError());
    s->pay_cur ^= 1;
    return PSIM_OK;
}

unsigned long long* phase_end_mark(psim_handle* h, Shard* s) {
    return h->cfg.manager == PSIM_MANAGER_PLUGGABLE ? nullptr
                                                    : reinterpret_cast<unsigned long long*>(s->stat_out.p + NST) + 1;
}

int route_group(psim_handle* h, Shard* s, bool dense, uint32_t m, bool fixed = false, bool exact = false) {
    const uint32_t n = s->n;
    uint32_t wshift = n > (1u << 26) ? 13 : n > (1u << 22) ? 12 : 11;
    if (const char* e = getenv("PSIM_ROUTE_WSHIFT")) {
        const int v = atoi(e);
        if (v >= (int)WSHIFT_MIN && v <= (int)WSHIFT_MAX) wshift = (uint32_t)v;
    }
    const uint32_t W = 1u << wshift, nb = (n + W - 1) >> wshift;
    const RouteIn in{s->outbox.p, s->okey.p, s->obase.p, s->ocnt.p, dense ? m : n, s->lo,
                     h->cfg.manager == PSIM_MANAGER_PLUGGABLE, dense ? s->recvh.p : nullptr,
                     dense ? s->recvt.p : nullptr, dense && !fixed ? s->wseg.p : nullptr, dense ? h->G : 0u,
                     fixed ? s->xcap_h : 0u, fixed ? s->xcap_t : 0u, (uint32_t)h->round};
    const uint32_t nsteps = std::max<uint32_t>(1, (in.n_src + RB_STEP - 1) / RB_STEP);
    const uint32_t nblk = std::min<uint32_t>(nsteps, h->rb_blocks);
    const size_t nh = (size_t)nb * nblk;
    TRY(s->hist.ensure(nh));
    TRY(s->hoff.ensure(nh));
    TRY(s->rtot.ensure(nb));
    TRY(s->rbase.ensure(nb + 1));
    static const bool lidx_ok = !getenv("PSIM_ROUTE_LIDX") || atoi(getenv("PSIM_ROUTE_LIDX")) != 0;
    const uint32_t lcap = lidx_ok && W == (1u << WSHIFT_MIN) ? ROUTE_LIDX : 0u;
    const size_t lds_h = (size_t)nb * 4, lds_r = (size_t)W * 16 + (size_t)lcap * 4;
    const uint32_t rows = s->pgrid + s->cgrid + s->rgrid + s->tgrid + s->sgrid + s->lgrid + s->qgrid + s->egrid;
    const StatsIn st{s->stat_part.p, rows,
                     fixed ? 0u : std::min<uint32_t>(nblk, std::min<uint32_t>(STAT_TILES, std::max<uint32_t>(1, rows / 32))),
                     s->stat_tile.p, s->stat_out.p, s->pin_dev + (size_t)s->stat_slot * PIN_STRIDE,
                     s->outx.p ? s->outx_top.p : nullptr, s->pin_dev};
    KTimer t(h, s, KT_SORT);
    if (!dense && !exact && h->route_fused && n <= (1u << 26)) {
        const uint64_t capb64 = (s->rcap + nb - 1) / nb * 3 / 2 + 64;
        const uint32_t capb = (uint32_t)std::min<uint64_t>(capb64, 0xFFFFFFFFull / nb);
        if (s->gcnt.n < nb) {
            TRY(s->gcnt.ensure(nb));
            HIP_TRY(hipMemsetAsync(s->gcnt.p, 0, s->gcnt.n * 4, s->stream));
        }
        TRY(s->pairs.ensure((size_t)nb * capb));
        TRY(s->rank.ensure((size_t)nb * capb));
        static const uint32_t walk = getenv("PSIM_FILL_WALK") && atoi(getenv("PSIM_FILL_WALK")) ? 1u : 0u;
        k_bucket_fill<false><<<nblk, RB_STEP, lds_h, s->stream>>>(in, nsteps, nb, wshift, s->gcnt.p, capb, s->pairs.p,
                                                                  s->ctl.p, phase_end_mark(h, s), st, walk);
        k_bucket_route<false><<<nb, RR_THREADS, lds_r, s->stream>>>(
            n, wshift, h->rr_reg, nullptr, s->pairs.p, in.rec, nullptr, nullptr, s->rank.p, s->cb.p, s->bmask.p,
            s->in_beg.p, s->ivals.p, s->tmp.p, s->inbox.p, s->pin_dev + PIN_M, s->rcap, s->ctl.p, s->gcnt.p, capb,
            s->batch_round1, st, lcap);
        HIP_TRY(hipGetLastError());
        return PSIM_OK;
    }
    if (dense)
        k_bucket_hist<true><<<nblk, RB_STEP, lds_h, s->stream>>>(in, nsteps, nb, wshift, s->hist.p, s->ctl.p,
                                                                 nullptr, st);
    else
        k_bucket_hist<false><<<nblk, RB_STEP, lds_h, s->stream>>>(in, nsteps, nb, wshift, s->hist.p, s->ctl.p,
                                                                  phase_end_mark(h, s), st);
    k_bucket_offsets<<<nb, RB_MAX_BLOCKS, 0, s->stream>>>(s->hist.p, nblk, s->hoff.p, s->rtot.p, s->ctl.p);
    if (dense)
        k_bucket_scatter<true><<<nblk, RB_STEP, lds_h, s->stream>>>(in, nsteps, nb, wshift, s->hoff.p, s->rtot.p,
                                                                    s->rbase.p, s->pairs.p, s->rcap,
                                                                    s->pin_dev + PIN_OVF, s->ctl.p,
                                                                    s->batch_round1, st);
    else
        k_bucket_scatter<false><<<nblk, RB_STEP, lds_h, s->stream>>>(in, nsteps, nb, wshift, s->hoff.p, s->rtot.p,
                                                                     s->rbase.p, s->pairs.p, s->rcap,
                                                                     s->pin_dev + PIN_OVF, s->ctl.p,
                                                                     s->batch_round1, st);
    if (dense)
        k_bucket_route<true><<<nb, RR_THREADS, lds_r, s->stream>>>(
            n, wshift, h->rr_reg, s->rbase.p, s->pairs.p, nullptr, in.wire, in.tails, s->rank.p, s->cb.p, s->bmask.p,
            s->in_beg.p, s->ivals.p, s->tmp.p, s->inbox.p, s->pin_dev + PIN_M, s->rcap, s->ctl.p, nullptr, 0u,
            s->batch_round1, st, lcap);
    else
        k_bucket_route<false><<<nb, RR_THREADS, lds_r, s->stream>>>(
            n, wshift, h->rr_reg, s->rbase.p, s->pairs.p, in.rec, nullptr, nullptr, s->rank.p, s->cb.p, s->bmask.p,
            s->in_beg.p, s->ivals.p, s->tmp.p, s->inbox.p, s->pin_dev + PIN_M, s->rcap, s->ctl.p, nullptr, 0u,
            s->batch_round1, st, lcap);
    HIP_TRY(hipGetLastError());
    return PSIM_OK;
}

int route_buffers(Shard* s, bool both_inboxes) {
    const size_t c = s->rcap + 1;
    TRY(s->ivals.ensure(c)); TRY(s->tmp.ensure(c)); TRY(s->rank.ensure(c)); TRY(s->pairs.ensure(c));
    (void)both_inboxes;
    TRY(s->inbox.ensure_keep(c, s->m_in, s->stream));
    return PSIM_OK;
}

int phase_route_local(psim_handle* h, Shard* s, bool exact = false) { return route_group(h, s, false, 0, false, exact); }

void send_counts(Shard* s, uint32_t G);

int phase_partition(psim_handle* h, Shard* s, bool fixed = false) {
    const uint32_t G = h->G;
    RouteIn in{};
    in.rec = s->outbox.p; in.okey = s->okey.p; in.obase = s->obase.p; in.ocnt = s->ocnt.p; in.n_src = s->n;
    const uint32_t nsteps = std::max<uint32_t>(1, (s->n + RB_STEP - 1) / RB_STEP);
    const uint32_t spb = (nsteps + h->rb_blocks - 1) / h->rb_blocks;
    const uint32_t nblk = (nsteps + spb - 1) / spb;
    const size_t nh = (size_t)2 * G * nblk + 1;
    TRY(s->hist.ensure(nh));
    TRY(s->hoff.ensure(nh));
    if (!fixed) TRY(s->sendbuf.ensure(2 * (s->pin[PIN_TOTAL] + 1), 2));
    TRY(s->d_off.ensure(2 * G + 1));
    const bool rccl = h->ranked;
    if (rccl) TRY(h->comm_cnt.ensure(2 * G + 2));
    s->soff.assign(2 * G + 1, 0);
    const uint32_t capH = fixed ? s->xcap_h : 0u, capT = fixed ? s->xcap_t : 0u;
    StatsIn st{};
    if (fixed) {
        const uint32_t rows = s->pgrid + s->cgrid + s->rgrid + s->tgrid + s->sgrid + s->lgrid + s->qgrid + s->egrid;
        st = StatsIn{s->stat_part.p, rows,
                     std::min<uint32_t>(nblk, std::min<uint32_t>(STAT_TILES, std::max<uint32_t>(1, rows / 32))),
                     s->stat_tile.p, s->stat_out.p, s->pin_dev + (size_t)s->stat_slot * PIN_STRIDE,
                     s->outx.p ? s->outx_top.p : nullptr, s->pin_dev};
    }
    {
        KTimer t(h, s, KT_SORT);
        k_owner_part<false><<<nblk, RB_STEP, 0, s->stream>>>(in, nsteps, spb, G, h->per, s->hist.p, nullptr,
                                                              nullptr, phase_end_mark(h, s), capH, capT, s->ctl.p, st);
        TRY(scan_excl(s, s->hist.p, s->hoff.p, (uint32_t)nh));
        k_owner_part<true><<<nblk, RB_STEP, 0, s->stream>>>(in, nsteps, spb, G, h->per, nullptr, s->hoff.p,
                                                             s->sendbuf.p, nullptr, capH, capT, s->ctl.p, StatsIn{});
        k_owner_offsets<<<1, OO_THREADS, 0, s->stream>>>(s->hoff.p, nblk, G, s->d_off.p, rccl ? h->comm_cnt.p : nullptr,
                                                  rccl ? s->stat_out.p + STAT_OUT_X : nullptr, capH, capT, s->ctl.p,
                                                  (uint32_t)h->round, s->idx, s->sendbuf.p, st);
        HIP_TRY(hipGetLastError());
        if (rccl) return PSIM_OK;
        HIP_TRY(hipMemcpyAsync(s->soff.data(), s->d_off.p, (2 * G + 1) * 8, hipMemcpyDeviceToHost, s->stream));
        TRY(stream_wait(s));
    }
    send_counts(s, G);
    return PSIM_OK;
}

void send_counts(Shard* s, uint32_t G) {
    s->scnt.resize(G);
    s->lcnt.resize(G);
    for (uint32_t g = 0; g < G; g++) {
        s->scnt[g] = s->soff[g + 1] - s->soff[g];
        s->lcnt[g] = s->soff[G + g + 1] - s->soff[G + g];
    }
}

int phase_receive(psim_handle* h, Shard* s, const std::vector<uint64_t>& hc, const std::vector<uint64_t>& lc) {
    const uint32_t G = h->G;
    s->wseg_host.assign(2 * (G + 1), 0);
    uint64_t m = 0, ml = 0;
    for (uint32_t g = 0; g < G; g++) {
        s->wseg_host[g] = (uint32_t)m;
        s->wseg_host[G + 1 + g] = (uint32_t)ml;
        m += hc[g];
        ml += lc[g];
    }
    s->wseg_host[G] = (uint32_t)m;
    s->wseg_host[2 * G + 1] = (uint32_t)ml;
    TRY(s->wseg.ensure(2 * (G + 1)));
    HIP_TRY(hipMemcpyAsync(s->wseg.p, s->wseg_host.data(), s->wseg_host.size() * 4, hipMemcpyHostToDevice,
                           s->stream));
    s->rcap = std::max<uint64_t>(s->rcap, m);
    TRY(route_buffers(s, false));
    TRY(route_group(h, s, true, (uint32_t)m));
    s->m_in = (uint32_t)m;
    return PSIM_OK;
}

int exchange_local(psim_handle* h) {
    const uint32_t G = h->G;
    for (Shard* d : h->shards) {
        std::vector<uint64_t> hc(G), lc(G);
        uint64_t m = 0, ml = 0;
        for (Shard* s : h->shards) {
            hc[s->idx] = s->scnt[d->idx];
            lc[s->idx] = s->lcnt[d->idx];
            m += hc[s->idx];
            ml += lc[s->idx];
        }
        TRY(d->recvh.ensure(m + 1));
        TRY(d->recvt.ensure(ml + 1));
        {
            KTimer t(h, d, KT_EXCHANGE);
            uint64_t oh = 0, ot = 0;
            for (uint32_t g = 0; g < G; g++) {
                Shard* s = h->shards[g];
                if (hc[g])
                    HIP_TRY(hipMemcpyAsync(d->recvh.p + oh, s->sendbuf.p + s->soff[d->idx], hc[g] * sizeof(Wire),
                                           hipMemcpyDeviceToDevice, d->stream));
                if (lc[g])
                    HIP_TRY(hipMemcpyAsync(d->recvt.p + ot, s->sendbuf.p + s->soff[G + d->idx], lc[g] * sizeof(Wire),
                                           hipMemcpyDeviceToDevice, d->stream));
                if (g != d->idx) {
                    h->x_records += hc[g];
                    h->x_bytes += (hc[g] + lc[g]) * sizeof(Wire);
                }
                oh += hc[g];
                ot += lc[g];
            }
        }
        TRY(phase_receive(h, d, hc, lc));
    }
    return PSIM_OK;
}

int exchange_rccl(psim_handle* h) {
    Shard* s = h->shards[0];
    const uint32_t G = h->G;
    std::vector<uint64_t> hc(G), lc(G);
    {
        KTimer t(h, s, KT_EXCHANGE);
        TRY(h->comm->all_to_all_u64(h->comm_cnt.p, h->comm_cnt.p + G, 1, s->stream));
        std::vector<uint64_t> rcnt(G);
        HIP_TRY(hipMemcpyAsync(rcnt.data(), h->comm_cnt.p + G, G * 8, hipMemcpyDeviceToHost, s->stream));
        HIP_TRY(hipMemcpyAsync(s->soff.data(), s->d_off.p, (2 * G + 1) * 8, hipMemcpyDeviceToHost, s->stream));
        TRY(stream_wait(s));
        send_counts(s, G);
        uint64_t m = 0, ml = 0;
        std::vector<uint64_t> roh(G), rot(G);
        for (uint32_t g = 0; g < G; g++) {
            hc[g] = rcnt[g] & 0xFFFFFFFFull;
            lc[g] = rcnt[g] >> 32;
            roh[g] = m;
            rot[g] = ml;
            m += hc[g];
            ml += lc[g];
        }
        TRY(s->recvh.ensure(m + 1));
        TRY(s->recvt.ensure(ml + 1));
        std::vector<Xfer> sends, recvs;
        const bool self_comm = h->world == 1;
        for (uint32_t g = 0; g < G; g++) {
            if (g == s->idx && !self_comm) continue;
            if (s->scnt[g]) sends.push_back({(int)g, s->sendbuf.p + s->soff[g], s->scnt[g] * sizeof(Wire)});
            if (s->lcnt[g]) sends.push_back({(int)g, s->sendbuf.p + s->soff[G + g], s->lcnt[g] * sizeof(Wire)});
            if (hc[g]) recvs.push_back({(int)g, s->recvh.p + roh[g], hc[g] * sizeof(Wire)});
            if (lc[g]) recvs.push_back({(int)g, s->recvt.p + rot[g], lc[g] * sizeof(Wire)});
            h->x_records += s->scnt[g];
            h->x_bytes += (s->scnt[g] + s->lcnt[g]) * sizeof(Wire);
        }
        TRY(h->comm->exchange(sends, recvs, s->stream));
        if (!self_comm) {
            const uint32_t g = s->idx;
            if (hc[g])
                HIP_TRY(hipMemcpyAsync(s->recvh.p + roh[g], s->sendbuf.p + s->soff[g], hc[g] * sizeof(Wire),
                                       hipMemcpyDeviceToDevice, s->stream));
            if (lc[g])
                HIP_TRY(hipMemcpyAsync(s->recvt.p + rot[g], s->sendbuf.p + s->soff[G + g], lc[g] * sizeof(Wire),
                                       hipMemcpyDeviceToDevice, s->stream));
        }
    }
    return phase_receive(h, s, hc, lc);
}

int exchange_fixed(psim_handle* h) {
    Shard* s = h->shards[0];
    const uint32_t G = h->G, capT = s->xcap_t;
    const size_t xs = XHDR + s->xcap_h;
    KTimer t(h, s, KT_EXCHANGE);
    std::vector<Xfer> sends, recvs;
    const bool self_comm = h->world == 1;
    for (uint32_t g = 0; g < G; g++) {
        if (g == s->idx && !self_comm) continue;
        sends.push_back({(int)g, s->sendbuf.p + g * xs, xs * sizeof(Wire)});
        sends.push_back({(int)g, s->sendbuf.p + G * xs + (size_t)g * capT, (size_t)capT * sizeof(Wire)});
        recvs.push_back({(int)g, s->recvh.p + g * xs, xs * sizeof(Wire)});
        recvs.push_back({(int)g, s->recvt.p + (size_t)g * capT, (size_t)capT * sizeof(Wire)});
    }
    TRY(h->comm->exchange(sends, recvs, s->stream));
    if (!self_comm) {
        const uint32_t g = s->idx;
        HIP_TRY(hipMemcpyAsync(s->recvh.p + g * xs, s->sendbuf.p + g * xs, xs * sizeof(Wire), hipMemcpyDeviceToDevice,
                               s->stream));
        HIP_TRY(hipMemcpyAsync(s->recvt.p + (size_t)g * capT, s->sendbuf.p + G * xs + (size_t)g * capT,
                               (size_t)capT * sizeof(Wire), hipMemcpyDeviceToDevice, s->stream));
    }
    return route_group(h, s, true, (uint32_t)(G * xs), true);
}

void xcaps_set(Shard* s, uint64_t mh, uint64_t mt, bool grow = false, bool shrink = true) {
    const uint64_t ch = std::min<uint64_t>(grow ? 2 * mh + 1024 : mh + mh / 2 + 1024, 0x7FFFFFFFull);
    const uint64_t ct = std::min<uint64_t>(grow ? 2 * mt + 1024 : mt + mt / 2 + 1024, 0x7FFFFFFFull);
    if (ch > s->xcap_h || (shrink && 2 * mh < s->xcap_h)) s->xcap_h = (uint32_t)ch;
    if (ct > s->xcap_t || (shrink && 2 * mt < s->xcap_t)) s->xcap_t = (uint32_t)ct;
}
void xcaps_max(psim_handle* h, const uint64_t* p, uint64_t& mh, uint64_t& mt) {
    for (int r = 0; r < h->world && r < 64; r++) {
        mh = std::max<uint64_t>(mh, p[PIN_XRANK + r]);
        mt = std::max<uint64_t>(mt, p[PIN_XRANK + 64 + r]);
    }
}
void xcaps_update(psim_handle* h, Shard* s, const uint64_t* p) {
    uint64_t mh = 0, mt = 0;
    xcaps_max(h, p, mh, mt);
    xcaps_set(s, mh, mt, false, false);
}

int phase_stats(psim_handle* h, Shard* s, const std::vector<uint32_t>& crashed, bool batched = false) {
    KTimer t(h, s, KT_STATS);
    if (h->ranked && !batched) {
        uint64_t* pw = s->pin_dev + (size_t)s->stat_slot * PIN_STRIDE;
        TRY(h->comm->all_reduce(s->stat_out.p, STAT_OUT_N, CType::U64, COp::SUM, s->stream));
        HIP_TRY(hipMemcpyAsync(pw, s->stat_out.p, NST * 8, hipMemcpyDeviceToDevice, s->stream));
        HIP_TRY(hipMemcpyAsync(pw + PIN_XRANK, s->stat_out.p + STAT_OUT_R, 128 * 8, hipMemcpyDeviceToDevice, s->stream));
    }
    if (!crashed.empty()) {
        TRY(upload(s, s->ev_ids, crashed));
        k_uncrash<<<grid_for(crashed.size()), BLK, 0, s->stream>>>(s->flags.p, s->crash_bits.p, s->ev_ids.p,
                                                                  (uint32_t)crashed.size(), s->ctl.p);
    }
    return PSIM_OK;
}

void bcast_slots(psim_handle* h, RoundCtl& ctl) {
    if (!h->pend_b_root.empty()) {
        for (size_t i = 0; i < h->pend_b_root.size(); i++) {
            const uint32_t k = h->pend_b_msg[i] % PSIM_MSG_SLOTS;
            ctl.bcast_clear |= 1ull << k;
            h->slot_tab[k] = h->pend_b_msg[i];
            h->slot_tab[PSIM_MSG_SLOTS + k] = h->pend_b_root[i] | PSIM_MAP_BIT;
        }
        h->tracked_msg = h->pend_b_msg.back();
    }
}

int run_round(psim_handle* h, uint64_t* st, bool events_applied = false, bool from_partition = false) {
    RoundCtl ctl;
    ctl.crashes = !h->pend_crash.empty();
    if (!events_applied) bcast_slots(h, ctl);
    if (h->faults_dirty) {
        if (h->nx_faulted.size() != h->N) h->nx_faulted.assign(h->N, 0);
        h->n_omit_s = (uint32_t)h->nx_omit_s.size();
        h->n_omit_r = (uint32_t)h->nx_omit_r.size();
        h->faults = h->n_omit_s || h->n_omit_r || h->nx_nfaulted;
    }
    for (Shard* s : h->shards) s->tn = 0;
    std::vector<RoundArgs> args(h->shards.size());
    for (size_t i = 0; i < h->shards.size() && !from_partition; i++)
        TRY(phase_events_prepare(h, h->shards[i], ctl, args[i], !events_applied, false, events_applied));
    static const long long fail_round = getenv("PSIM_TEST_FAIL_ROUND") ? atoll(getenv("PSIM_TEST_FAIL_ROUND")) : -1;
    if (fail_round >= 0 && h->round == (uint64_t)fail_round) {
        for (Shard* s : h->shards) (void)hipStreamSynchronize(s->stream);
        return PSIM_ENOMEM;
    }
    for (size_t i = 0; i < h->shards.size() && !from_partition; i++) TRY(phase_consume(h, h->shards[i], args[i]));
    if (local_route(h)) {
        TRY(phase_route_local(h, h->shards[0]));
    } else {
        for (Shard* s : h->shards) TRY(phase_partition(h, s));
        if (h->ranked) TRY(exchange_rccl(h));
        else TRY(exchange_local(h));
    }
    for (Shard* s : h->shards) {
        TRY(phase_stats(h, s, h->pend_crash));
        if (!h->pend_b_root.empty())
            k_origin<<<grid_for(h->pend_b_root.size()), BLK, 0, s->stream>>>(
                s->origin.p, s->lo, s->n, s->bc_roots.p, s->bc_msgs.p, (uint32_t)h->pend_b_root.size(), s->flags.p,
                true, s->ctl.p);
    }
    memset(st, 0, NST * 8);
    for (Shard* s : h->shards) {
        TRY(stream_wait(s));
        flush_timers(h, s);
        for (int k = 0; k < NST; k++) st[k] += s->pin[k];
        if (local_route(h) && s->pin[PIN_OVF]) {
            const uint64_t m = s->pin[PIN_OVF];
            s->pin[PIN_OVF] = 0;
            if (s->rcap < m + m / 2) {
                const uint64_t want = m + m / 2;
                if (want <= (1ull << 26)) while (s->rcap < want) s->rcap <<= 1;
                else s->rcap = (want + (1ull << 20) - 1) >> 20 << 20;
            }
            TRY(route_buffers(s, false));
            TRY(phase_route_local(h, s, true));
            TRY(stream_wait(s));
        }
        if (local_route(h)) s->m_in = (uint32_t)s->pin[PIN_M];
        if (h->ranked) xcaps_update(h, s, s->pin);
        static const bool trace_relay = getenv("PSIM_TRACE_RELAY") != nullptr;
        if (trace_relay && s->rgrid)
        {
            uint64_t em = 0;
            for (int k = 0; k < ST_NTYPES; k++) em += s->pin[ST_EMIT + k];
            std::fprintf(stderr, "psim: round %llu shard %u: %u nodes with work, %u to k_consume, %u to k_pt, "
                         "%u to k_shuf, %u to k_consume_lite, %u to k_ptl, outbox bound %llu, emitted %llu\n",
                         (unsigned long long)h->round, s->idx, read1(s, s->d_nact.p), read1(s, s->n_slow.p),
                         read1(s, s->n_pt.p), read1(s, s->n_shuf.p), read1(s, s->n_lite.p) + read1(s, s->n_lite.p + 1) + read1(s, s->n_lite.p + 2) + read1(s, s->n_lite.p + 3),
                         read1(s, s->n_ptl.p) + read1(s, s->n_ptl.p + 1) + read1(s, s->n_ptl.p + 2) + read1(s, s->n_ptl.p + 3),
                         (unsigned long long)s->pin[PIN_TOTAL], (unsigned long long)em);
        }
        if (s->pin[NST] != ~0ull && s->pin[NST + 1] > s->pin[NST]) {
            h->kt_ms[KT_CONSUME] += (double)(s->pin[NST + 1] - s->pin[NST]) * 1e-5;
            h->kt_n[KT_CONSUME]++;
        }
    }
    if (st[ST_BOUND]) {
        std::fprintf(stderr, "psim: round %llu: %llu nodes emitted past their outbox bound (engine bug)\n",
                     (unsigned long long)h->round, (unsigned long long)st[ST_BOUND]);
        return PSIM_EDEVICE;
    }
    for (uint32_t j : h->pend_join) h->pend_join_mark[j] = 0;
    h->pend_crash.clear(); h->pend_join.clear(); h->pend_contact.clear();
    h->pend_lv_a.clear(); h->pend_lv_t.clear();
    if (st[ST_STOP]) {
        std::vector<uint32_t> ids;
        for (Shard* s : h->shards) {
            const size_t k = read1(s, s->n_stop.p);
            if (!k) continue;
            const size_t at = ids.size();
            ids.resize(at + k);
            HIP_TRY(hipMemcpyAsync(ids.data() + at, s->stop_ids.p, k * 4, hipMemcpyDeviceToHost, s->stream));
            TRY(stream_wait(s));
        }
        if (h->ranked) {
            Shard* s = h->shards[0];
            const uint32_t W = h->world;
            std::vector<uint64_t> cnt(W), mine(ids.begin(), ids.end());
            const uint64_t k = mine.size();
            TRY(h->comm_cnt.ensure(W + 1));
            HIP_TRY(hipMemcpyAsync(h->comm_cnt.p + W, &k, 8, hipMemcpyHostToDevice, s->stream));
            TRY(h->comm->all_gather(h->comm_cnt.p + W, h->comm_cnt.p, 8, s->stream));
            HIP_TRY(hipMemcpyAsync(cnt.data(), h->comm_cnt.p, W * 8, hipMemcpyDeviceToHost, s->stream));
            TRY(stream_wait(s));
            const uint64_t mk = *std::max_element(cnt.begin(), cnt.end());
            mine.resize(mk, 0);
            std::vector<uint64_t> all((size_t)W * mk);
            TRY(h->comm_cnt.ensure((size_t)W * mk + mk));
            HIP_TRY(hipMemcpyAsync(h->comm_cnt.p + (size_t)W * mk, mine.data(), mk * 8, hipMemcpyHostToDevice,
                                   s->stream));
            TRY(h->comm->all_gather(h->comm_cnt.p + (size_t)W * mk, h->comm_cnt.p, mk * 8, s->stream));
            HIP_TRY(hipMemcpyAsync(all.data(), h->comm_cnt.p, all.size() * 8, hipMemcpyDeviceToHost, s->stream));
            TRY(stream_wait(s));
            ids.clear();
            for (uint32_t r = 0; r < W; r++)
                for (uint64_t j = 0; j < cnt[r]; j++) ids.push_back((uint32_t)all[(size_t)r * mk + j]);
        }
        std::sort(ids.begin(), ids.end());
        h->pend_crash.insert(h->pend_crash.end(), ids.begin(), ids.end());
    }
    h->pend_part_set = h->pend_part_clear = false;
    h->faults_dirty = false;
    h->pend_b_root.clear(); h->pend_b_msg.clear();
    h->round++;
    return PSIM_OK;
}

void fill_stats(const uint64_t* s, uint64_t round, psim_round_stats* o) {
    memset(o, 0, sizeof *o);
    o->round = round;
    for (int i = 0; i < ST_NTYPES; i++) {
        o->emitted[i] = s[ST_EMIT + i];
        o->delivered[i] = s[ST_DELIV + i];
    }
    o->dropped = s[ST_DROPPED]; o->nodes_up = s[ST_UP]; o->nodes_processed = s[ST_PROC];
    o->exits = s[ST_EXITS]; o->send_fail = s[ST_FAIL]; o->first_deliveries = s[ST_FIRST];
    o->overflow = s[ST_OVF]; o->digest = s[ST_DIGEST]; o->state_bytes = s[ST_BYTES];
    for (int k = 0; k < PSIM_OVF_NKINDS; k++) o->overflow_by[k] = s[ST_OVF_BY + k];
    o->omitted = s[ST_OMIT];
}

bool batchable(psim_handle* h) {
    static const bool trace = getenv("PSIM_TRACE_RELAY") != nullptr;
    static const bool off = getenv("PSIM_NO_BATCH") != nullptr || getenv("PSIM_TEST_FAIL_ROUND") != nullptr;
    static const bool off_ranked = getenv("PSIM_NO_RANK_BATCH") != nullptr;
    if (off || trace || h->phase_timers || h->cfg.strict || h->cfg.manager == PSIM_MANAGER_PLUGGABLE ||
        !h->pend_lv_a.empty())
        return false;
    Shard* s = h->shards[0];
    if (h->ranked) return !off_ranked && s->reserved && s->outbox.n && s->xcap_h && s->xcap_t;
    return h->G == 1 && s->reserved && s->rcap && s->outbox.n;
}

uint64_t batch_desc_cap(const psim_handle* h, const Shard* s) {
    static const struct Hook {
        uint64_t slots = 0;
        long rank = -1;
        Hook() {
            const char* e = getenv("PSIM_TEST_DESC_CAP");
            if (!e) return;
            slots = strtoull(e, nullptr, 10);
            if (const char* at = strchr(e, '@')) rank = atol(at + 1);
        }
    } hook;
    const uint64_t real = std::min<uint64_t>(s->outbox.n, s->okey.n);
    if (!hook.slots || (hook.rank >= 0 && hook.rank != h->rank)) return real;
    return std::min<uint64_t>(real, hook.slots);
}

int run_batch(psim_handle* h, uint32_t nb, psim_round_stats* st_out, uint32_t* done_out) {
    Shard* s = h->shards[0];
    const uint64_t r0 = h->round;
    RoundCtl ctl0;
    ctl0.crashes = !h->pend_crash.empty();
    bcast_slots(h, ctl0);
    const std::vector<uint32_t> crashed0 = h->pend_crash;
    const std::vector<uint32_t> none;
    const bool bc0 = !h->pend_b_root.empty();
    s->tn = 0;
    s->desc_cap = batch_desc_cap(h, s);
    const auto t_enq = std::chrono::steady_clock::now();
    for (uint32_t j = 0; j < nb; j++) {
        s->stat_slot = j + 1;
        s->batch_round1 = (uint32_t)h->round + 1;
        RoundArgs a;
        const RoundCtl ctl = j == 0 ? ctl0 : RoundCtl{};
        TRY(phase_events_prepare(h, s, ctl, a, j == 0, true));
        TRY(phase_consume(h, s, a));
        TRY(phase_route_local(h, s));
        TRY(phase_stats(h, s, j == 0 ? crashed0 : none));
        if (j == 0 && bc0)
            k_origin<<<grid_for(h->pend_b_root.size()), BLK, 0, s->stream>>>(
                s->origin.p, s->lo, s->n, s->bc_roots.p, s->bc_msgs.p, (uint32_t)h->pend_b_root.size(), s->flags.p,
                true, s->ctl.p);
        HIP_TRY(hipGetLastError());
        h->round++;
    }
    s->stat_slot = 0; s->batch_round1 = 0; s->desc_cap = 0;
    uint32_t cw[2] = {0, 0};
    HIP_TRY(hipMemcpyAsync(cw, s->ctl.p, sizeof cw, hipMemcpyDeviceToHost, s->stream));
    const auto t_wait = std::chrono::steady_clock::now();
    TRY(stream_wait(s));
    static const bool trace_batch = getenv("PSIM_TRACE_BATCH") != nullptr;
    if (trace_batch)
        std::fprintf(stderr, "psim: batch of %u from round %llu: enqueue %.3f ms, wait %.3f ms\n", nb,
                     (unsigned long long)r0, std::chrono::duration<double, std::milli>(t_wait - t_enq).count(),
                     std::chrono::duration<double, std::milli>(std::chrono::steady_clock::now() - t_wait).count());
    if (s->pin[PIN_BIGIN]) {
        s->pin[PIN_BIGIN] = 0;
        HIP_TRY(hipMemsetAsync(s->ctl.p, 0, sizeof cw, s->stream));
        return PSIM_ENOMEM;
    }
    const uint32_t done = cw[0] ? (uint32_t)(cw[1] - r0) : nb;
    if (cw[0] && (cw[1] < r0 || done >= nb)) return PSIM_EDEVICE;
    for (uint32_t j = 0; j < done; j++) {
        const uint64_t* p = s->pin + (size_t)(j + 1) * PIN_STRIDE;
        if (p[ST_BOUND]) {
            std::fprintf(stderr, "psim: round %llu: %llu nodes emitted past their outbox bound (engine bug)\n",
                         (unsigned long long)(r0 + j), (unsigned long long)p[ST_BOUND]);
            return PSIM_EDEVICE;
        }
        if (st_out) fill_stats(p, r0 + j, &st_out[j]);
        if (p[NST] != ~0ull && p[NST + 1] > p[NST]) {
            h->kt_ms[KT_CONSUME] += (double)(p[NST + 1] - p[NST]) * 1e-5;
            h->kt_n[KT_CONSUME]++;
        }
    }
    if (done > 0) {
        for (uint32_t j : h->pend_join) h->pend_join_mark[j] = 0;
        h->pend_crash.clear(); h->pend_join.clear(); h->pend_contact.clear();
        h->pend_part_set = h->pend_part_clear = false;
        h->pend_b_root.clear(); h->pend_b_msg.clear();
        h->faults_dirty = false;
    }
    s->m_in = (uint32_t)s->pin[PIN_M];
    *done_out = done;
    if (!cw[0]) {
        h->round = r0 + nb;
        return PSIM_OK;
    }
    HIP_TRY(hipMemsetAsync(s->ctl.p, 0, sizeof cw, s->stream));
    h->round = r0 + done;
    uint64_t st[NST];
    if (cw[0] == 1) {
        const uint64_t total = s->pin[PIN_TOTAL];
        if (total >= 0xFFFFFFFFull) return PSIM_ENOMEM;
        std::fprintf(stderr, "psim: round %llu: outbox grows past its capacity (%zu -> %llu slots)\n",
                     (unsigned long long)h->round, s->outbox.n, (unsigned long long)total + 1);
        TRY(s->outbox.ensure(total + 1, 2));
        TRY(s->okey.ensure(total + 1, 2));
        TRY(stream_wait(s));
        TRY(run_round(h, st, done == 0));
    } else {
        const uint64_t m = s->pin[PIN_OVF];
        s->pin[PIN_OVF] = 0;
        const uint64_t want = m + m / 2;
        if (want <= (1ull << 26)) while (s->rcap < want) s->rcap <<= 1;
        else s->rcap = (want + (1ull << 20) - 1) >> 20 << 20;
        TRY(route_buffers(s, false));
        TRY(phase_route_local(h, s, true));
        TRY(phase_stats(h, s, done == 0 ? crashed0 : none));
        if (done == 0 && bc0)
            k_origin<<<grid_for(h->pend_b_root.size()), BLK, 0, s->stream>>>(
                s->origin.p, s->lo, s->n, s->bc_roots.p, s->bc_msgs.p, (uint32_t)h->pend_b_root.size(), s->flags.p,
                true, s->ctl.p);
        TRY(stream_wait(s));
        for (int k = 0; k < NST; k++) st[k] = s->pin[k];
        if (st[ST_BOUND]) return PSIM_EDEVICE;
        s->m_in = (uint32_t)s->pin[PIN_M];
        if (s->pin[NST] != ~0ull && s->pin[NST + 1] > s->pin[NST]) {
            h->kt_ms[KT_CONSUME] += (double)(s->pin[NST + 1] - s->pin[NST]) * 1e-5;
            h->kt_n[KT_CONSUME]++;
        }
        if (done == 0) {
            for (uint32_t j : h->pend_join) h->pend_join_mark[j] = 0;
            h->pend_crash.clear(); h->pend_join.clear(); h->pend_contact.clear();
            h->pend_part_set = h->pend_part_clear = false;
            h->pend_b_root.clear(); h->pend_b_msg.clear();
            h->faults_dirty = false;
        }
        h->round++;
    }
    if (st_out) fill_stats(st, r0 + done, &st_out[done]);
    *done_out = done + 1;
    return PSIM_OK;
}

int run_batch_ranked(psim_handle* h, uint32_t nb, psim_round_stats* st_out, uint32_t* done_out) {
    Shard* s = h->shards[0];
    const uint32_t G = h->G, capH = s->xcap_h, capT = s->xcap_t;
    const uint64_t r0 = h->round;
    TRY(s->sendbuf.ensure((size_t)G * (XHDR + capH + capT) + 1));
    TRY(s->recvh.ensure((size_t)G * (XHDR + capH) + 1));
    TRY(s->recvt.ensure((size_t)G * capT + 1));
    TRY(h->comm_cnt.ensure(2 * G + 2));
    s->rcap = std::max<uint64_t>(s->rcap, (uint64_t)G * capH);
    TRY(route_buffers(s, false));
    RoundCtl ctl0;
    ctl0.crashes = !h->pend_crash.empty();
    bcast_slots(h, ctl0);
    const std::vector<uint32_t> crashed0 = h->pend_crash;
    const std::vector<uint32_t> none;
    const bool bc0 = !h->pend_b_root.empty();
    s->tn = 0;
    s->desc_cap = batch_desc_cap(h, s);
    const auto t_enq = std::chrono::steady_clock::now();
    double tph[5] = {0, 0, 0, 0, 0};
    auto tick = [](std::chrono::steady_clock::time_point& t0, double& acc) {
        const auto t1 = std::chrono::steady_clock::now();
        acc += std::chrono::duration<double, std::milli>(t1 - t0).count();
        t0 = t1;
    };
    for (uint32_t j = 0; j < nb; j++) {
        s->stat_slot = j + 1;
        s->batch_round1 = (uint32_t)h->round + 1;
        RoundArgs a;
        const RoundCtl ctl = j == 0 ? ctl0 : RoundCtl{};
        auto t0 = std::chrono::steady_clock::now();
        TRY(phase_events_prepare(h, s, ctl, a, j == 0, true));
        tick(t0, tph[0]);
        TRY(phase_consume(h, s, a));
        tick(t0, tph[1]);
        TRY(phase_partition(h, s, true));
        tick(t0, tph[2]);
        TRY(exchange_fixed(h));
        tick(t0, tph[3]);
        TRY(phase_stats(h, s, j == 0 ? crashed0 : none, true));
        tick(t0, tph[4]);
        if (j == 0 && bc0)
            k_origin<<<grid_for(h->pend_b_root.size()), BLK, 0, s->stream>>>(
                s->origin.p, s->lo, s->n, s->bc_roots.p, s->bc_msgs.p, (uint32_t)h->pend_b_root.size(), s->flags.p,
                true, s->ctl.p);
        HIP_TRY(hipGetLastError());
        h->round++;
    }
    s->stat_slot = 0; s->batch_round1 = 0; s->desc_cap = 0;
    uint32_t cw[2] = {0, 0};
    HIP_TRY(hipMemcpyAsync(cw, s->ctl.p, sizeof cw, hipMemcpyDeviceToHost, s->stream));
    const auto t_wait = std::chrono::steady_clock::now();
    TRY(stream_wait(s));
    const auto t_end = std::chrono::steady_clock::now();
    if (s->pin[PIN_BIGIN]) {
        s->pin[PIN_BIGIN] = 0;
        HIP_TRY(hipMemsetAsync(s->ctl.p, 0, sizeof cw, s->stream));
        return PSIM_ENOMEM;
    }
    uint32_t done = nb;
    for (uint32_t j = 0; j < nb; j++)
        if (s->pin[(size_t)(j + 1) * PIN_STRIDE + PIN_XAB]) { done = j; break; }
    if (done == nb && cw[0]) return PSIM_EDEVICE;
    {
        uint64_t mh = 0, mt = 0;
        for (uint32_t j = 0; j <= done && j < nb; j++) xcaps_max(h, s->pin + (size_t)(j + 1) * PIN_STRIDE, mh, mt);
        xcaps_set(s, mh, mt, done < nb);
    }
    static const bool trace_batch = getenv("PSIM_TRACE_BATCH") != nullptr;
    if (trace_batch)
        std::fprintf(stderr, "psim: rank %d: batch of %u from round %llu: %u done%s; caps %u heads, %u tails; "
                     "enqueue %.3f ms (prepare %.3f, node phase %.3f, partition %.3f, exchange + route %.3f, end "
                     "%.3f), wait %.3f ms\n",
                     h->rank, nb, (unsigned long long)r0, done, done < nb ? " (one redone exactly)" : "", s->xcap_h,
                     s->xcap_t, std::chrono::duration<double, std::milli>(t_wait - t_enq).count(), tph[0], tph[1],
                     tph[2], tph[3], tph[4], std::chrono::duration<double, std::milli>(t_end - t_wait).count());
    const bool self_comm = h->world == 1;
    for (uint32_t j = 0; j < done; j++) {
        const uint64_t* p = s->pin + (size_t)(j + 1) * PIN_STRIDE;
        if (p[ST_BOUND]) {
            std::fprintf(stderr, "psim: round %llu: %llu nodes emitted past their outbox bound (engine bug)\n",
                         (unsigned long long)(r0 + j), (unsigned long long)p[ST_BOUND]);
            return PSIM_EDEVICE;
        }
        if (st_out) fill_stats(p, r0 + j, &st_out[j]);
        if (p[NST] != ~0ull && p[NST + 1] > p[NST]) {
            h->kt_ms[KT_CONSUME] += (double)(p[NST + 1] - p[NST]) * 1e-5;
            h->kt_n[KT_CONSUME]++;
        }
        for (uint32_t g = 0; g < G; g++) {
            if (g == s->idx && !self_comm) continue;
            h->x_records += p[PIN_XCNT + g] & 0xFFFFFFFFull;
            h->x_bytes += (uint64_t)(XHDR + capH + capT) * sizeof(Wire);
        }
    }
    if (done > 0) {
        for (uint32_t j : h->pend_join) h->pend_join_mark[j] = 0;
        h->pend_crash.clear(); h->pend_join.clear(); h->pend_contact.clear();
        h->pend_part_set = h->pend_part_clear = false;
        h->pend_b_root.clear(); h->pend_b_msg.clear();
        h->faults_dirty = false;
    }
    s->m_in = (uint32_t)s->pin[PIN_M];
    *done_out = done;
    if (done == nb) {
        h->round = r0 + nb;
        s->xbatch = std::min<uint32_t>(2 * s->xbatch, BATCH_MAX);
        return PSIM_OK;
    }
    s->xbatch = std::max<uint32_t>(2, s->xbatch / 4);
    HIP_TRY(hipMemsetAsync(s->ctl.p, 0, sizeof cw, s->stream));
    h->round = r0 + done;
    const bool short_outbox = cw[0] == 1 && cw[1] == (uint32_t)h->round;
    uint64_t st[NST];
    if (short_outbox) {
        std::fprintf(stderr, "psim: round %llu: outbox grows past its capacity (%zu -> %llu slots)\n",
                     (unsigned long long)h->round, s->outbox.n, (unsigned long long)s->pin[PIN_TOTAL] + 1);
        TRY(stream_wait(s));
    }
    TRY(run_round(h, st, done == 0, !short_outbox));
    if (st_out) fill_stats(st, r0 + done, &st_out[done]);
    *done_out = done + 1;
    return PSIM_OK;
}

int shard_alloc(psim_handle* h, Shard* s) {
    HIP_TRY(hipStreamCreateWithFlags(&s->stream, hipStreamNonBlocking));
    HIP_TRY(hipEventCreateWithFlags(&s->wait_ev, hipEventDisableTiming));
    for (int k = 0; k < 2; k++) {
        HIP_TRY(hipStreamCreateWithFlags(&s->side[k], hipStreamNonBlocking));
        HIP_TRY(hipEventCreateWithFlags(&s->join_ev[k], hipEventDisableTiming));
    }
    HIP_TRY(hipEventCreateWithFlags(&s->fork_ev, hipEventDisableTiming));
    if (s->n > (1u << 26)) {
        HIP_TRY(hipFuncSetAttribute((const void*)k_bucket_route<false>, hipFuncAttributeMaxDynamicSharedMemorySize,
                                    8192 * 16));
        HIP_TRY(hipFuncSetAttribute((const void*)k_bucket_route<true>, hipFuncAttributeMaxDynamicSharedMemorySize,
                                    8192 * 16));
    }
    HIP_TRY(hipHostMalloc((void**)&s->pin, (size_t)PIN_STRIDE * (1 + BATCH_MAX) * sizeof(uint64_t), hipHostMallocMapped));
    HIP_TRY(hipHostGetDevicePointer((void**)&s->pin_dev, s->pin, 0));
    memset(s->pin, 0, (size_t)PIN_STRIDE * (1 + BATCH_MAX) * sizeof(uint64_t));
    for (int k = 0; k < Shard::MAXT; k++) {
        HIP_TRY(hipEventCreate(&s->ev[k][0]));
        HIP_TRY(hipEventCreate(&s->ev[k][1]));
    }
    s->ev_live = true;
    const size_t N = h->N, n = std::max<uint32_t>(s->n, 1);
    int rc = 0;
    rc |= s->flags.alloc(N); rc |= s->part.alloc(N); rc |= s->hdr.alloc(n);
    if (h->cfg.manager != PSIM_MANAGER_PLUGGABLE) { rc |= s->upart.alloc(N); rc |= s->lite_cm.alloc(n); }
    rc |= s->crash_bits.alloc((N >> (CRASH_GRAIN_SHIFT + 5)) + 1);
    rc |= s->act.alloc(n * PSIM_ACTIVE_CAP); rc |= s->pas.alloc(n * PSIM_PASSIVE_CAP);
    rc |= s->sentm.alloc(n * IDMAP_IN); rc |= s->recvm.alloc(n * IDMAP_IN);
    if (h->cfg.manager != PSIM_MANAGER_PLUGGABLE) {
        const size_t rows = h->cfg.manager == PSIM_MANAGER_XBOT ? 2 * n : std::max<size_t>(1024, n / 32);
        rc |= s->mapx.alloc(rows * IDMAP_EXT);
    }
    rc |= s->mapx_top.alloc(1);
    rc |= s->pt_all.alloc(n * PSIM_PT_MEMBERS_CAP); rc |= s->pt_com.alloc(n * PSIM_PT_MEMBERS_CAP);
    rc |= s->pt_eag.alloc(n * RT_SET); rc |= s->pt_laz.alloc(n * RT_SET); rc |= s->pt_rt.alloc(n * RT_WORDS);
    rc |= s->origin.alloc(n); rc |= s->slots.alloc(2 * PSIM_MSG_SLOTS);
    rc |= s->pt_out.alloc(n * OUT_IN); rc |= s->start.alloc(n);
    if (h->cfg.manager != PSIM_MANAGER_PLUGGABLE) rc |= s->conn.alloc(n * PSIM_CONN_CAP);
    if (h->cfg.manager != PSIM_MANAGER_PLUGGABLE) {
        size_t rows = std::max<size_t>(1024, n / 8);
        if (const char* e = getenv("PSIM_OUTX_ROWS")) rows = std::max<size_t>(1, (size_t)atoll(e));
        rc |= s->outx.alloc(rows * OUT_EXT);
    }
    rc |= s->outx_top.alloc(1);
    rc |= s->ocnt.alloc(n); rc |= s->cb.alloc(n + 1);
    rc |= s->in_beg.alloc(n + 1); rc |= s->bound.alloc(n + 1); rc |= s->pscan.alloc(4097); rc |= s->obase.alloc(n + 1);
    rc |= s->bmask.alloc(n); rc |= s->btot.alloc(4096);
    rc |= s->desc.alloc(n); rc |= s->d_nact.alloc(1);
    rc |= s->desc_slow.alloc(n); rc |= s->n_slow.alloc(1);
    rc |= s->desc_pt.alloc(n); rc |= s->n_pt.alloc(1);
    rc |= s->desc_shuf.alloc(n); rc |= s->n_shuf.alloc(1);
    rc |= s->desc_lite.alloc(2 * n); rc |= s->n_lite.alloc(4);
    rc |= s->desc_ptl.alloc(2 * n); rc |= s->n_ptl.alloc(4);
    if (h->cfg.manager == PSIM_MANAGER_PLUGGABLE) { rc |= s->stop_ids.alloc(n); rc |= s->n_stop.alloc(1); }
    rc |= s->stat_out.alloc(STAT_OUT_N);
    rc |= s->ctl.alloc(4);
    rc |= s->stat_tile.alloc((size_t)STAT_TILES * NST);
    rc |= s->ikeys.alloc(1024); rc |= s->ivals.alloc(1024);
    rc |= s->recvh.alloc(1024); rc |= s->recvt.alloc(1024); rc |= s->wseg.alloc(130); rc |= s->inbox.alloc(1024); rc |= s->outbox.alloc(1024);
    if (h->cfg.manager == PSIM_MANAGER_PLUGGABLE) {
        if (h->cfg.strategy == PSIM_STRATEGY_FULL) {
            rc |= s->fbits.alloc(n * 2 * h->fw);
            rc |= s->pay_top.alloc(1);
            rc |= s->pay[0].alloc(2 * h->fw); rc |= s->pay[1].alloc(2 * h->fw);
        } else {
            rc |= s->sview.alloc(n * PSIM_SVIEW_CAP);
            if (h->cfg.strategy == PSIM_STRATEGY_SCAMP_V2) rc |= s->sinv.alloc(n * PSIM_SVIEW_CAP);
        }
    }
    if (rc) return PSIM_ENOMEM;
    HIP_TRY(hipDeviceSynchronize());
    return PSIM_OK;
}

void shard_free(Shard* s) {
    if (s->stream) (void)hipStreamSynchronize(s->stream);
    s->flags.release(); s->part.release(); s->upart.release(); s->lite_cm.release(); s->hdr.release(); s->crash_bits.release(); s->btab.release();
    s->act.release(); s->pas.release(); s->sentm.release(); s->recvm.release();
    s->pt_all.release(); s->pt_com.release();
    s->mapx.release(); s->mapx_top.release();
    s->pt_eag.release(); s->pt_laz.release(); s->pt_out.release(); s->start.release(); s->conn.release();
    s->outx.release(); s->outx_top.release();
    s->pt_rt.release(); s->origin.release(); s->slots.release(); s->bc_roots.release(); s->bc_msgs.release();
    s->ikeys.release(); s->ivals.release(); s->recvh.release(); s->recvt.release(); s->wseg.release(); s->inbox.release();
    if (s->pin) (void)hipHostFree(s->pin);
    if (s->wait_ev) (void)hipEventDestroy(s->wait_ev);
    s->wait_ev = nullptr;
    for (int k = 0; k < 2; k++) {
        if (s->join_ev[k]) (void)hipEventDestroy(s->join_ev[k]);
        if (s->side[k]) (void)hipStreamDestroy(s->side[k]);
        s->join_ev[k] = nullptr;
        s->side[k] = nullptr;
    }
    if (s->fork_ev) (void)hipEventDestroy(s->fork_ev);
    s->fork_ev = nullptr;
    s->pin = nullptr;
    s->outbox.release(); s->okey.release(); s->ocnt.release();
// ... 1050 lines not shown
```

### profiles/round_kernels.py

```python
import csv
import re
import sys

rows = sorted(csv.DictReader(open(sys.argv[1])), key=lambda r: int(r["Start_Timestamp"]))
steps = int(sys.argv[2]) if len(sys.argv) > 2 and not sys.argv[2].startswith("--") else 60
tail = int(sys.argv[sys.argv.index("--tail") + 1]) if "--tail" in sys.argv else 0
rounds, cur = [], None
for r in rows:
    name = re.sub(r"\(.*", "", r["Kernel_Name"].replace("(anonymous namespace)::", "")).replace("void ", "").strip()
    d = (int(r["End_Timestamp"]) - int(r["Start_Timestamp"])) / 1e3
    if "k_node_prep" in name:
        cur = {"_start": int(r["Start_Timestamp"])}
        rounds.append(cur)
    if cur is not None:
        cur[name] = cur.get(name, 0.0) + d
        cur["_end"] = int(r["End_Timestamp"])
rounds = rounds[:-1]
if tail:
    rounds = rounds[:-tail]
last = rounds[-steps:]
tot = {}
for c in last:
    for k, v in c.items():
        if not k.startswith("_"):
            tot[k] = tot.get(k, 0.0) + v / len(last)
span = sum((c["_end"] - c["_start"]) / 1e3 for c in last) / len(last)
busy = sum(tot.values())
print(f"{len(last)} rounds: kernel time {busy / 1e3:.2f} ms/round, first-to-last kernel span {span / 1e3:.2f} ms/round")
for k, v in sorted(tot.items(), key=lambda kv: -kv[1]):
    print(f"  {v / 1e3:9.3f} ms  {v / busy * 100:5.1f} %  {k}")
```

Before: 2.881 billion.

## Fuse next round's HyParView node prepare into the bucket route kernel

For the HyParView/Plumtree path, the per-node bound computation of the following round (hv_node_prep) now runs inside k_bucket_route, right after that kernel has produced the per-node counts and broadcast masks. The route kernel writes packed bounds, per-range sums and stat partials, and the separate k_node_prep launch is skipped for that round. The aim is to avoid re-reading cb/bmask and one kernel launch per round. In exchange it adds LDS, registers and a launch-bounds occupancy hint to the route kernel. It applies only at the minimum window shift, with no crashes in the round, and with a power-of-two prep range size.

```diff
diff --git a/partisan_amd/csrc/psim_engine.hip b/partisan_amd/csrc/psim_engine.hip
--- a/partisan_amd/csrc/psim_engine.hip
+++ b/partisan_amd/csrc/psim_engine.hip
@@ -756,17 +756,187 @@
     return p < 2 || wire_long(tt) ? v : make_uint4(0, 0, 0, 0);
 }
 
-template <bool WIRE>
-__global__ void __launch_bounds__(RR_THREADS) k_bucket_route(
+constexpr uint64_t NODE_STATE_BYTES = 416;
+
+__device__ __forceinline__ bool due(uint32_t period, uint32_t r, uint32_t start) {
+    return period > 0 && r > start && ((r - start) % period) == 0;
+}
+
+#ifdef PSIM_BOUND_TERMS
+enum { BT_RESP, BT_TIMER, BT_PUSH, BT_PUSH_NE, BT_NPUSH, BT_LAZY, BT_ON, BT_NL, BT_LC, BT_CRASH, BT_XBOT,
+       BT_BUMP, BT_TOTAL, BT_C, BT_QUIET, BT_ROUNDS, BT_N };
+__device__ unsigned long long g_bterm[BT_N];
+#define BTERM(k, v) (bt[k] += (v))
+#define BT_PARAM , unsigned long long* bt
+#define BT_ARG , bt
+#else
+#define BTERM(k, v) ((void)0)
+#define BT_PARAM
+#define BT_ARG
+#endif
+
+struct PrepSums {
+    unsigned long long up, drop, bs, ws, qp, qf;
+};
+
+template <bool EVENTS, class A>
+__device__ __forceinline__ uint64_t hv_node_prep(const A& a, uint32_t i, uint8_t f, unsigned long long cbi,
+                                                 unsigned long long bm_, uint32_t st, uint32_t org_,
+                                                 PrepSums& s BT_PARAM) {
+    uint64_t b = 0;
+    uint32_t w = 0;
+    const uint32_t c = (uint32_t)cbi;
+    if (f & F_UP) {
+        const uint32_t r = a.round;
+        bool origin = org_ != 0;
+        const Hdr& x = a.hdr[i];
+        const bool promo = a.random_promotion && due(a.promotion_period, r, st);
+        b = (cbi >> 32) + (st == r && x.join_contact != PSIM_NONE ? 1u : 0u) + (promo ? 1u : 0u) +
+            (due(a.shuffle_period, r, st) ? 1u : 0u);
+        BTERM(BT_RESP, cbi >> 32);
+        BTERM(BT_TIMER, b - (cbi >> 32));
+        const unsigned long long bm = c ? bm_ : 0ull;
+        const uint32_t pushes = (uint32_t)__popcll(bm) + (origin ? 1u : 0u);
+        const bool lazy = a.plumtree && due(a.lazy_tick_period, r, st);
+        uint32_t lazy_add = 0, push_sum = 0, union_sum = 0;
+        if (pushes) {
+            const uint4 r0 = *reinterpret_cast<const uint4*>(a.pt_rt + (size_t)i * RT_WORDS);
+            const uint2 cn = *reinterpret_cast<const uint2*>(a.pt_rt + (size_t)i * RT_WORDS + RT_EN);
+            const uint32_t rts[4] = {r0.x, r0.y, r0.z, r0.w};
+            auto push = [&](uint32_t root) {
+                uint32_t ne = PSIM_PT_MEMBERS_CAP, nl = 0, ne0 = 0;
+#pragma unroll
+                for (int k = 0; k < PSIM_PT_ROOTS; k++)
+                    if (rts[k] == root) {
+                        ne0 = (cn.x >> (8 * k)) & 0xFFu;
+                        ne = max(ne, ne0);
+                        nl = (cn.y >> (8 * k)) & 0xFFu;
+                    }
+                const uint32_t pb = min(2u * PSIM_ACTIVE_CAP, ne + c);
+                push_sum += pb;
+                lazy_add += nl + c;
+                union_sum += min(pb + nl + c, max((uint32_t)PSIM_PT_MEMBERS_CAP, ne0 + nl) + c);
+                BTERM(BT_PUSH, min(2u * PSIM_ACTIVE_CAP, ne + c));
+                BTERM(BT_PUSH_NE, min(2u * PSIM_ACTIVE_CAP, ne));
+                BTERM(BT_NPUSH, 1);
+                BTERM(BT_NL, nl);
+                BTERM(BT_LC, c);
+            };
+            for (unsigned long long m = bm; m; m &= m - 1) push(a.slots[PSIM_MSG_SLOTS + __ffsll(m) - 1]);
+            if (origin) push((a.lo + i) | PSIM_MAP_BIT);
+        }
+        if (lazy) {
+            const uint32_t fo = (uint32_t)f >> F_OUTN_SHIFT;
+            const uint32_t on = fo < 15 ? fo : (uint32_t)x.out_n;
+            const uint32_t pl = min(push_sum + min((uint32_t)PSIM_PT_OUT_CAP, on + lazy_add), on + union_sum);
+            b += pl;
+            BTERM(BT_LAZY, pl - push_sum);
+            BTERM(BT_ON, on);
+        } else {
+            b += push_sum;
+        }
+        if (pushes) BTERM(BT_C, c);
+        bool exits = false;
+        bool lazy_wake = false;
+        if constexpr (EVENTS) {
+            lazy_wake = a.lazy_wake;
+            if (a.crash_round) {
+                const uint4* ar = reinterpret_cast<const uint4*>(a.act + (size_t)i * PSIM_ACTIVE_CAP);
+                const uint4 a0 = ar[0], a1 = ar[1];
+                const uint32_t av[8] = {a0.x, a0.y, a0.z, a0.w, a1.x, a1.y, a1.z, a1.w};
+                uint32_t cv[PSIM_CONN_CAP] = {};
+                const uint32_t cn = x.conn_n;
+                if (cn) {
+                    const uint4* cr = reinterpret_cast<const uint4*>(a.conn + (size_t)i * PSIM_CONN_CAP);
+                    const uint4 c0 = cr[0], c1 = cr[1];
+                    cv[0] = c0.x; cv[1] = c0.y; cv[2] = c0.z; cv[3] = c0.w;
+                    cv[4] = c1.x; cv[5] = c1.y; cv[6] = c1.z; cv[7] = c1.w;
+                }
+#pragma unroll
+                for (int k = 0; k < PSIM_ACTIVE_CAP; k++)
+                    if ((uint32_t)k < x.act_n && av[k] < a.n_nodes && av[k] != a.lo + i &&
+                        crashed_now(a, av[k])) {
+                        b++;
+                        BTERM(BT_CRASH, 1);
+                        bool down = false;
+#pragma unroll
+                        for (int j = 0; j < PSIM_CONN_CAP; j++) down |= (uint32_t)j < cn && cv[j] == (av[k] | PSIM_CONN_DOWN);
+                        exits |= !down;
+                    }
+#pragma unroll
+                for (int j = 0; j < PSIM_CONN_CAP; j++)
+                    exits |= (uint32_t)j < cn && !(cv[j] & PSIM_CONN_DOWN) && crashed_now(a, cv[j] & KEY_DST_MASK);
+            }
+        }
+        const uint32_t fon = (uint32_t)f >> F_OUTN_SHIFT;
+        const bool quiet_ok = a.lazy_tick_period == 1 && !lazy_wake && !(f & F_LAZY);
+        w = c > 0 || st == r || exits || (fon && !quiet_ok) || origin ||
+            (a.random_promotion && (f & F_LOWACT) && due(a.promotion_period, r, st)) ||
+            due(a.shuffle_period, r, st);
+        if (a.xbot) {
+            const bool xb = due(a.xbot_period, r, st);
+            const uint32_t cl = x.conn_cl;
+            b += (xb ? 2u : 0u) + cl;
+            BTERM(BT_XBOT, (xb ? 2u : 0u) + cl);
+            w = w || xb || cl;
+        }
+        if (w && b == 0) { b = 1; BTERM(BT_BUMP, 1); }
+        if (!w && fon && lazy) {
+            s.qp++;
+            s.qf += fon < 15 ? fon : (uint32_t)x.out_n;
+            BTERM(BT_QUIET, 1);
+            b = 0;
+        }
+        s.up++;
+    } else {
+        s.drop += c;
+    }
+    s.bs += b;
+    s.ws += w;
+    BTERM(BT_TOTAL, b);
+    return (b << 32) | w;
+}
+
+struct RoutePrep {
+    uint32_t round, n_nodes, lo;
+    uint32_t shuffle_period, promotion_period, random_promotion, plumtree, lazy_tick_period, xbot, xbot_period;
+    uint32_t pshift, nranges;
+    const uint8_t* flags;
+    const Hdr* hdr;
+    const uint32_t *pt_rt, *slots, *start;
+    uint64_t* packed;
+    uint32_t* ocnt;
+    uint64_t* tiles;
+    unsigned long long* btot;
+    uint64_t* part;
+};
+constexpr uint32_t RP_NODES = (1u << WSHIFT_MIN) / RR_THREADS;
+static_assert(RP_NODES == 2, "k_bucket_route's prepare holds the first two nodes' words");
+constexpr uint32_t RP_RANGES = (1u << WSHIFT_MAX) / BLK;
+enum { RP_BLO, RP_BHI, RP_UP, RP_W, RP_QP, RP_DROP, RP_QF, RP_N = 8 };
+static_assert((1u << WSHIFT_MIN) * 16 + ROUTE_LIDX * 4 + (PSIM_RR_THREADS + 4) * 4 + RP_RANGES * RP_N * 4 + 256 <= 80 * 1024,
+              "k_bucket_route at W = 2^11 with the prepare's range sums: two blocks a CU");
+
+__device__ __forceinline__ uint32_t wave_sum(uint32_t v) {
+#pragma unroll
+    for (int o = 32; o > 0; o >>= 1) v += __shfl_xor(v, o);
+    return v;
+}
+__device__ __forceinline__ uint32_t wave_sum_rare(uint32_t v) { return __ballot(v != 0) ? wave_sum(v) : 0u; }
+
+template <bool WIRE, bool PREP = false>
+__global__ void __launch_bounds__(RR_THREADS, 8) k_bucket_route(
     uint32_t n, uint32_t wshift, uint32_t regcap, const uint32_t* __restrict__ base,
     const uint2* __restrict__ pairs, const Msg* __restrict__ rec, const Wire* __restrict__ heads,
     const Wire* __restrict__ tails, uint32_t* rank, unsigned long long* cb,
     unsigned long long* bmask, uint32_t* in_beg, uint32_t* idx, uint32_t* tmp, Msg* __restrict__ inbox, uint64_t* hm,
-    uint64_t cap, uint32_t* ctl, const uint32_t* gcnt, uint32_t capb, uint32_t round1, StatsIn st, uint32_t lcap) {
+    uint64_t cap, uint32_t* ctl, const uint32_t* gcnt, uint32_t capb, uint32_t round1, StatsIn st, uint32_t lcap,
+    RoutePrep rp) {
     if (*ctl) return;
     extern __shared__ __attribute__((aligned(16))) uint32_t sm[];
     __shared__ __attribute__((aligned(16))) uint32_t spart[RR_THREADS + 4];
     uint32_t& s_nl = spart[RR_THREADS];
+    __shared__ __attribute__((aligned(8))) uint32_t s_rp[RP_RANGES][RP_N];
     const uint32_t W = 1u << wshift, wmask = W - 1, b = blockIdx.x;
     uint32_t* cnt = sm;
     uint32_t* bs = sm + W;
@@ -803,6 +973,17 @@
     }
     pairs += q0;
     rank += q0;
+    constexpr bool prep = PREP && !WIRE;
+    uint8_t pf[RP_NODES] = {};
+    uint32_t pst[RP_NODES] = {};
+    if (prep) {
+#pragma unroll
+        for (uint32_t k = 0; k < RP_NODES; k++) {
+            const uint32_t d = (b << wshift) + threadIdx.x + k * RR_THREADS;
+            if (d < n) { pf[k] = rp.flags[rp.lo + d]; pst[k] = rp.start[d]; }
+        }
+        for (uint32_t j = threadIdx.x; j < RP_RANGES * RP_N; j += blockDim.x) (&s_rp[0][0])[j] = 0;
+    }
     uint32_t* const ix = lcap && s1 - s0 <= lcap ? sm + 4 * W : idx + s0;
     for (uint32_t j = threadIdx.x; j < 4 * W; j += blockDim.x) sm[j] = 0;
     if (threadIdx.x == 0) s_nl = 0;
@@ -843,11 +1024,18 @@
         uint32_t tot;
         spart[threadIdx.x] = block_excl<uint32_t, RR_THREADS>(sum, &tot) + sum;
     }
-    for (uint32_t dl = threadIdx.x; dl < W; dl += blockDim.x) {
+    uint32_t pbs[RP_NODES] = {};
+    unsigned long long pmk[RP_NODES] = {};
+    for (uint32_t dl = threadIdx.x, k = 0; dl < W; dl += blockDim.x, k++) {
         const uint32_t d = (b << wshift) + dl;
         if (d >= n) break;
-        cb[d] = cnt[dl] | ((unsigned long long)bs[dl] << 32);
-        bmask[d] = mk[dl];
+        const uint32_t bv = bs[dl];
+        const unsigned long long mv = mk[dl];
+        cb[d] = cnt[dl] | ((unsigned long long)bv << 32);
+        bmask[d] = mv;
+        if (prep) {
+            if (k == 0) { pbs[0] = bv; pmk[0] = mv; } else { pbs[RP_NODES - 1] = bv; pmk[RP_NODES - 1] = mv; }
+        }
     }
     __syncthreads();
     uint32_t run = spart[threadIdx.x] - sum;
@@ -877,6 +1065,45 @@
         }
     }
     __syncthreads();
+#ifndef PSIM_BOUND_TERMS
+    if (prep) {
+        uint64_t pk[RP_NODES];
+#pragma unroll
+        for (uint32_t k = 0; k < RP_NODES; k++) {
+            const uint32_t dl = threadIdx.x + k * RR_THREADS, d = (b << wshift) + dl;
+            PrepSums ps{0, 0, 0, 0, 0, 0};
+            pk[k] = 0;
+            if (d < n)
+                pk[k] = hv_node_prep<false>(rp, d, pf[k], cnt[dl] | ((unsigned long long)pbs[k] << 32), pmk[k], pst[k],
+                                            0u, ps);
+            const uint32_t uwq = wave_sum((uint32_t)ps.up | (uint32_t)ps.ws << 10 | (uint32_t)ps.qp << 20);
+            const uint32_t drop = wave_sum_rare((uint32_t)ps.drop), qf = wave_sum_rare((uint32_t)ps.qf);
+            const uint32_t blo = wave_sum((uint32_t)ps.bs & 0xFFFFFFu);
+            const unsigned long long bhi = (unsigned long long)wave_sum_rare((uint32_t)(ps.bs >> 24) & 0xFFFFFFu) +
+                                           ((unsigned long long)wave_sum_rare((uint32_t)(ps.bs >> 48)) << 24);
+            if ((threadIdx.x & 63) == 0) {
+                uint32_t* row = s_rp[dl >> rp.pshift];
+                if (uwq) {
+                    atomicAdd(&row[RP_UP], uwq & 0x3FFu);
+                    atomicAdd(&row[RP_W], (uwq >> 10) & 0x3FFu);
+                    atomicAdd(&row[RP_QP], uwq >> 20);
+                }
+                if (drop) atomicAdd(&row[RP_DROP], drop);
+                if (qf) atomicAdd(&row[RP_QF], qf);
+                const unsigned long long bsum = blo + (bhi << 24);
+                if (bsum) atomicAdd(reinterpret_cast<unsigned long long*>(&row[RP_BLO]), bsum);
+            }
+        }
+#pragma unroll
+        for (uint32_t k = 0; k < RP_NODES; k++) {
+            const uint32_t d = (b << wshift) + threadIdx.x + k * RR_THREADS;
+            if (d < n) {
+                rp.packed[d] = pk[k];
+                rp.ocnt[d] = 0;
+            }
+        }
+    }
+#endif
     uint32_t* sv = reinterpret_cast<uint32_t*>(mk);
     uint32_t* ll = sv + RUN_LDS;
     for (uint32_t dl = threadIdx.x; dl < W; dl += blockDim.x) {
@@ -904,6 +1131,24 @@
             if (t < k) q[t] = v[t];
     }
     __syncthreads();
+    if (prep) {
+        const uint32_t nrb = max(1u, W >> rp.pshift), c = threadIdx.x & 63;
+        for (uint32_t j = threadIdx.x >> 6; j < nrb; j += blockDim.x >> 6) {
+            const uint32_t R = ((b << wshift) >> rp.pshift) + j;
+            if (R >= rp.nranges) break;
+            const uint64_t up = s_rp[j][RP_UP], ws = s_rp[j][RP_W], qp = s_rp[j][RP_QP];
+            const unsigned long long bsum = *reinterpret_cast<const unsigned long long*>(&s_rp[j][RP_BLO]);
+            if (c == 0) {
+                rp.tiles[R] = ((uint64_t)bsum << 32) + ws;
+                rp.btot[R] = bsum;
+                if (R == rp.nranges - 1) rp.tiles[rp.nranges] = 0;
+            }
+            if (c < NST)
+                rp.part[(size_t)R * NST + c] = c == ST_UP ? up : c == ST_DROPPED ? (uint64_t)s_rp[j][RP_DROP]
+                                             : c == ST_PROC ? qp : c == ST_FAIL ? (uint64_t)s_rp[j][RP_QF]
+                                             : c == ST_BYTES ? ws * (2 * NODE_STATE_BYTES) : 0ull;
+        }
+    }
     const uint32_t nl = s_nl, wv = threadIdx.x >> 6, nwv = blockDim.x >> 6;
     for (uint32_t q = wv; q < nl; q += nwv) {
         const uint32_t dl = ll[q], k = cnt[dl];
@@ -930,21 +1175,6 @@
         if (t2 < m4) reinterpret_cast<uint4*>(&inbox[s0 + (t2 >> 2)])[t2 & 3] = c;
     }
 }
-
-constexpr uint64_t NODE_STATE_BYTES = 416;
-
-__device__ __forceinline__ bool due(uint32_t period, uint32_t r, uint32_t start) {
-    return period > 0 && r > start && ((r - start) % period) == 0;
-}
-
-#ifdef PSIM_BOUND_TERMS
-enum { BT_RESP, BT_TIMER, BT_PUSH, BT_PUSH_NE, BT_NPUSH, BT_LAZY, BT_ON, BT_NL, BT_LC, BT_CRASH, BT_XBOT,
-       BT_BUMP, BT_TOTAL, BT_C, BT_QUIET, BT_ROUNDS, BT_N };
-__device__ unsigned long long g_bterm[BT_N];
-#define BTERM(k, v) (bt[k] += (v))
-#else
-#define BTERM(k, v) ((void)0)
-#endif
 
 __global__ void __launch_bounds__(BLK) k_node_prep(RoundArgs a, const unsigned long long* bmask, uint64_t* packed,
                                                    uint64_t* part, uint32_t* ocnt, unsigned long long* btot,
@@ -965,8 +1195,7 @@
     if (a.upart && a.upart_dirty)
         for (uint32_t g = blockIdx.x * blockDim.x + threadIdx.x; g < a.n_nodes; g += gridDim.x * blockDim.x)
             a.upart[g] = (a.flags[g] & F_UP) ? (upart_t)a.part[g] : UPART_DOWN;
-    unsigned long long up = 0, drop = 0, bs = 0, ws = 0;
-    unsigned long long qp = 0, qf = 0;
+    PrepSums ps{0, 0, 0, 0, 0, 0};
 #ifdef PSIM_BOUND_TERMS
     unsigned long long bt[BT_N] = {};
 #endif
@@ -989,133 +1218,31 @@
         return q;
     };
     auto node = [&](uint32_t i, const PrepIn& cur) -> uint64_t {
-        uint8_t f = cur.f;
+        if (!a.pl) return hv_node_prep<true>(a, i, cur.f, cur.cbi, cur.bm, cur.st, cur.org, ps BT_ARG);
         uint64_t b = 0;
         uint32_t w = 0;
-        const unsigned long long cbi = cur.cbi;
-        uint32_t c = (uint32_t)cbi;
-        const uint32_t st_ = cur.st;
-        const uint32_t org_ = cur.org;
-        const unsigned long long bm_ = cur.bm;
-        if (f & F_UP) {
-            uint32_t st = st_, r = a.round;
-            if (a.pl) {
-                const Hdr& x = a.hdr[i];
-                bool pending = x.join_contact != PSIM_NONE;
-                bool per = due(a.periodic, r, st);
-                bool leave = x.pad1[0] != 0;
-                if (a.strategy == PSIM_STRATEGY_FULL)
-                    b = a.fanout ? (uint64_t)c + a.fanout + 1
-                                 : ((uint64_t)c + 2 + (leave ? 1 : 0)) * (a.n_nodes + 1);
-                else
-                {
-                    const uint64_t vn = x.act_n, vg = vn + c + 1;
-                    b = (uint64_t)c + (pending ? 1 + 2 * vg : 0) + (per ? 1 + vg : 0) + (leave ? vn : 0) + 1;
-                }
-                w = c > 0 || (pending && !x.have) || per || leave;
-            } else {
-                bool origin = org_ != 0;
-                const Hdr& x = a.hdr[i];
-                const bool promo = a.random_promotion && due(a.promotion_period, r, st);
-                b = (cbi >> 32) + (st == r && x.join_contact != PSIM_NONE ? 1u : 0u) + (promo ? 1u : 0u) +
-                    (due(a.shuffle_period, r, st) ? 1u : 0u);
-                BTERM(BT_RESP, cbi >> 32);
-                BTERM(BT_TIMER, b - (cbi >> 32));
-                const unsigned long long bm = c ? bm_ : 0ull;
-                const uint32_t pushes = (uint32_t)__popcll(bm) + (origin ? 1u : 0u);
-                const bool lazy = a.plumtree && due(a.lazy_tick_period, r, st);
-                uint32_t lazy_add = 0, push_sum = 0, union_sum = 0;
-                if (pushes) {
-                    const uint4 r0 = *reinterpret_cast<const uint4*>(a.pt_rt + (size_t)i * RT_WORDS);
-                    const uint2 cn = *reinterpret_cast<const uint2*>(a.pt_rt + (size_t)i * RT_WORDS + RT_EN);
-                    const uint32_t rts[4] = {r0.x, r0.y, r0.z, r0.w};
-                    auto push = [&](uint32_t root) {
-                        uint32_t ne = PSIM_PT_MEMBERS_CAP, nl = 0, ne0 = 0;
-#pragma unroll
-                        for (int k = 0; k < PSIM_PT_ROOTS; k++)
-                            if (rts[k] == root) {
-                                ne0 = (cn.x >> (8 * k)) & 0xFFu;
-                                ne = max(ne, ne0);
-                                nl = (cn.y >> (8 * k)) & 0xFFu;
-                            }
-                        const uint32_t pb = min(2u * PSIM_ACTIVE_CAP, ne + c);
-                        push_sum += pb;
-                        lazy_add += nl + c;
-                        union_sum += min(pb + nl + c, max((uint32_t)PSIM_PT_MEMBERS_CAP, ne0 + nl) + c);
-                        BTERM(BT_PUSH, min(2u * PSIM_ACTIVE_CAP, ne + c));
-                        BTERM(BT_PUSH_NE, min(2u * PSIM_ACTIVE_CAP, ne));
-                        BTERM(BT_NPUSH, 1);
-                        BTERM(BT_NL, nl);
-                        BTERM(BT_LC, c);
-                    };
-                    for (unsigned long long m = bm; m; m &= m - 1) push(a.slots[PSIM_MSG_SLOTS + __ffsll(m) - 1]);
-                    if (origin) push((a.lo + i) | PSIM_MAP_BIT);
-                }
-                if (lazy) {
-                    const uint32_t fo = (uint32_t)f >> F_OUTN_SHIFT;
-                    const uint32_t on = fo < 15 ? fo : (uint32_t)x.out_n;
-                    const uint32_t pl = min(push_sum + min((uint32_t)PSIM_PT_OUT_CAP, on + lazy_add), on + union_sum);
-                    b += pl;
-                    BTERM(BT_LAZY, pl - push_sum);
-                    BTERM(BT_ON, on);
-                } else {
-                    b += push_sum;
-                }
-                if (pushes) BTERM(BT_C, c);
-                bool exits = false;
-                if (a.crash_round) {
-                    const uint4* ar = reinterpret_cast<const uint4*>(a.act + (size_t)i * PSIM_ACTIVE_CAP);
-                    const uint4 a0 = ar[0], a1 = ar[1];
-                    const uint32_t av[8] = {a0.x, a0.y, a0.z, a0.w, a1.x, a1.y, a1.z, a1.w};
-                    uint32_t cv[PSIM_CONN_CAP] = {};
-                    const uint32_t cn = x.conn_n;
-                    if (cn) {
-                        const uint4* cr = reinterpret_cast<const uint4*>(a.conn + (size_t)i * PSIM_CONN_CAP);
-                        const uint4 c0 = cr[0], c1 = cr[1];
-                        cv[0] = c0.x; cv[1] = c0.y; cv[2] = c0.z; cv[3] = c0.w;
-                        cv[4] = c1.x; cv[5] = c1.y; cv[6] = c1.z; cv[7] = c1.w;
-                    }
-#pragma unroll
-                    for (int k = 0; k < PSIM_ACTIVE_CAP; k++)
-                        if ((uint32_t)k < x.act_n && av[k] < a.n_nodes && av[k] != a.lo + i &&
-                            crashed_now(a, av[k])) {
-                            b++;
-                            BTERM(BT_CRASH, 1);
-                            bool down = false;
-#pragma unroll
-                            for (int j = 0; j < PSIM_CONN_CAP; j++) down |= (uint32_t)j < cn && cv[j] == (av[k] | PSIM_CONN_DOWN);
-                            exits |= !down;
-                        }
-#pragma unroll
-                    for (int j = 0; j < PSIM_CONN_CAP; j++)
-                        exits |= (uint32_t)j < cn && !(cv[j] & PSIM_CONN_DOWN) && crashed_now(a, cv[j] & KEY_DST_MASK);
-                }
-                const uint32_t fon = (uint32_t)f >> F_OUTN_SHIFT;
-                const bool quiet_ok = a.lazy_tick_period == 1 && !a.lazy_wake && !(f & F_LAZY);
-                w = c > 0 || st == r || exits || (fon && !quiet_ok) || origin ||
-                    (a.random_promotion && (f & F_LOWACT) && due(a.promotion_period, r, st)) ||
-                    due(a.shuffle_period, r, st);
-                if (a.xbot) {
-                    const bool xb = due(a.xbot_period, r, st);
-                    const uint32_t cl = x.conn_cl;
-                    b += (xb ? 2u : 0u) + cl;
-                    BTERM(BT_XBOT, (xb ? 2u : 0u) + cl);
-                    w = w || xb || cl;
-                }
-                if (w && b == 0) { b = 1; BTERM(BT_BUMP, 1); }
-                if (!w && fon && lazy) {
-                    qp++;
-                    qf += fon < 15 ? fon : (uint32_t)x.out_n;
-                    BTERM(BT_QUIET, 1);
-                    b = 0;
-                }
+        const uint32_t c = (uint32_t)cur.cbi;
+        if (cur.f & F_UP) {
+            const uint32_t st = cur.st, r = a.round;
+            const Hdr& x = a.hdr[i];
+            bool pending = x.join_contact != PSIM_NONE;
+            bool per = due(a.periodic, r, st);
+            bool leave = x.pad1[0] != 0;
+            if (a.strategy == PSIM_STRATEGY_FULL)
+                b = a.fanout ? (uint64_t)c + a.fanout + 1
+                             : ((uint64_t)c + 2 + (leave ? 1 : 0)) * (a.n_nodes + 1);
+            else
+            {
+                const uint64_t vn = x.act_n, vg = vn + c + 1;
+                b = (uint64_t)c + (pending ? 1 + 2 * vg : 0) + (per ? 1 + vg : 0) + (leave ? vn : 0) + 1;
             }
-            up++;
+            w = c > 0 || (pending && !x.have) || per || leave;
+            ps.up++;
         } else {
-            drop += c;
-        }
-        bs += b;
-        ws += w;
+            ps.drop += c;
+        }
+        ps.bs += b;
+        ps.ws += w;
         BTERM(BT_TOTAL, b);
         return (b << 32) | w;
     };
@@ -1152,20 +1279,20 @@
     }
 #endif
     for (int o = 32; o > 0; o >>= 1) {
-        up += __shfl_xor(up, o);
-        drop += __shfl_xor(drop, o);
-        bs += __shfl_xor(bs, o);
-        ws += __shfl_xor(ws, o);
-        qp += __shfl_xor(qp, o);
-        qf += __shfl_xor(qf, o);
+        ps.up += __shfl_xor(ps.up, o);
+        ps.drop += __shfl_xor(ps.drop, o);
+        ps.bs += __shfl_xor(ps.bs, o);
+        ps.ws += __shfl_xor(ps.ws, o);
+        ps.qp += __shfl_xor(ps.qp, o);
+        ps.qf += __shfl_xor(ps.qf, o);
     }
     if ((threadIdx.x & 63) == 0) {
-        if (up) atomicAdd(&s_up, up);
-        if (drop) atomicAdd(&s_drop, drop);
-        if (bs) atomicAdd(&s_b, bs);
-        if (ws) atomicAdd(&s_w, ws);
-        if (qp) atomicAdd(&s_qp, qp);
-        if (qf) atomicAdd(&s_qf, qf);
+        if (ps.up) atomicAdd(&s_up, ps.up);
+        if (ps.drop) atomicAdd(&s_drop, ps.drop);
+        if (ps.bs) atomicAdd(&s_b, ps.bs);
+        if (ps.ws) atomicAdd(&s_w, ps.ws);
+        if (ps.qp) atomicAdd(&s_qp, ps.qp);
+        if (ps.qf) atomicAdd(&s_qf, ps.qf);
     }
     __syncthreads();
     if (threadIdx.x == 0) {
@@ -1245,8 +1372,20 @@
                                                   const uint32_t* __restrict__ start, RoundArgs a,
                                                   uint4* __restrict__ desc, uint64_t* __restrict__ obase,
                                                   uint32_t* nact, const unsigned long long* btot,
-                                                  uint32_t nranges, uint64_t* hout, uint64_t cap, uint32_t* ctl) {
+                                                  uint32_t nranges, uint64_t* hout, uint64_t cap, uint32_t* ctl,
+                                                  uint32_t* gcnt, uint32_t ngcnt) {
     if (*ctl) return;
+    if (gcnt) {
+        for (uint32_t j = blockIdx.x * blockDim.x + threadIdx.x; j < ngcnt; j += gridDim.x * blockDim.x) gcnt[j] = 0;
+        if (blockIdx.x == 0 && threadIdx.x == 0) {
+            ctl[2] = 0;
+            a.ktime[0] = ~0ull; a.ktime[1] = 0; *a.n_slow = 0; *a.n_pt = 0;
+            if (a.n_shuf) *a.n_shuf = 0;
+            if (a.n_lite) { a.n_lite[0] = 0; a.n_lite[1] = 0; a.n_lite[2] = 0; a.n_lite[3] = 0; }
+            if (a.n_ptl) { a.n_ptl[0] = 0; a.n_ptl[1] = 0; a.n_ptl[2] = 0; a.n_ptl[3] = 0; }
+            if (a.n_stop) *a.n_stop = 0;
+        }
+    }
     const bool last = blockIdx.x == gridDim.x - 1;
     const uint32_t r0 = blockIdx.x * DESC_RANGES;
     const uint32_t i0 = r0 * per, i1 = min(a.n_local, i0 + DESC_RANGES * per);
@@ -1774,6 +1913,8 @@
     uint64_t desc_cap = 0;
     uint32_t batch_round1 = 0;
     uint32_t stat_slot = 0;
+    uint32_t prep_next = 0;
+    bool prepared = false;
     bool outx_short = false;
     uint32_t xcap_h = 0, xcap_t = 0;
     uint32_t xbatch = 1;
@@ -1837,6 +1978,31 @@
         return x >= 0 && x <= 2 ? x : PTL_EARLY_DEFAULT;
     }();
     return v;
+}
+
+constexpr int PREP_FUSED_DEFAULT = 1;
+bool prep_fused_knob() {
+#ifdef PSIM_BOUND_TERMS
+    return false;
+#else
+    static const bool v = [] {
+        const char* e = getenv("PSIM_PREP_FUSED");
+        return e && *e ? atoi(e) != 0 : PREP_FUSED_DEFAULT != 0;
+    }();
+    return v;
+#endif
+}
+
+uint32_t route_wshift(uint32_t n) {
+    uint32_t wshift = n > (1u << 26) ? 13 : n > (1u << 22) ? 12 : 11;
+    static const int env = getenv("PSIM_ROUTE_WSHIFT") ? atoi(getenv("PSIM_ROUTE_WSHIFT")) : 0;
+    if (env >= (int)WSHIFT_MIN && env <= (int)WSHIFT_MAX) wshift = (uint32_t)env;
+    return wshift;
+}
+
+bool prep_fused_handle(const psim_handle* h, const Shard* s) {
+    return prep_fused_knob() && h->G == 1 && !h->ranked && h->route_fused && s->n <= (1u << 26) &&
+           h->cfg.manager != PSIM_MANAGER_PLUGGABLE;
 }
 
 RoundArgs make_args(psim_handle* h, Shard* s) {
@@ -2009,10 +2175,11 @@
     return PSIM_OK;
 }
 
-int scan_desc(Shard* s, const RoundArgs& a) {
+int scan_desc(Shard* s, const RoundArgs& a, bool resets = false) {
     k_desc<<<(s->pgrid + DESC_RANGES - 1) / DESC_RANGES, PREP_BLK, 0, s->stream>>>(
         s->bound.p, s->pscan.p, s->pper, s->in_beg.p, s->cb.p, s->start.p, a, s->desc.p, s->obase.p, s->d_nact.p,
-        s->btot.p, s->pgrid, s->pin_dev, s->desc_cap, s->ctl.p);
+        s->btot.p, s->pgrid, s->pin_dev, s->desc_cap, s->ctl.p, resets ? s->gcnt.p : nullptr,
+        resets ? (uint32_t)s->gcnt.n : 0u);
     HIP_TRY(hipGetLastError());
     return PSIM_OK;
 }
@@ -2051,7 +2218,7 @@
 };
 
 int phase_events_prepare(psim_handle* h, Shard* s, const RoundCtl& ctl, RoundArgs& a, bool events = true,
-                         bool batched = false, bool redo = false) {
+                         bool batched = false, bool redo = false, bool prepared = false) {
     const uint32_t n = s->n;
     if (events && h->faults_dirty) {
         std::vector<uint64_t> keys(h->nx_omit_s.begin(), h->nx_omit_s.end());
@@ -2110,6 +2277,8 @@
         {
             const uint32_t g = std::min<uint32_t>(std::max<uint32_t>(1, grid_for(n) / PREP_NPT), DESC_RANGES * PREP_BLK);
             s->pper = BLK * (uint32_t)(((uint64_t)n + (uint64_t)g * BLK - 1) / ((uint64_t)g * BLK));
+            if (prep_fused_handle(h, s))
+                while (s->pper & (s->pper - 1)) s->pper += s->pper & (0u - s->pper);
             s->pgrid = std::max<uint32_t>(1, (uint32_t)(((uint64_t)n + s->pper - 1) / s->pper));
         }
         s->cgrid = std::min<uint32_t>(grid_for(n), h->consume_blocks);
@@ -2124,9 +2293,10 @@
         s->egrid = ptl_early_knob() ? s->qgrid : 0;
         TRY(s->stat_part.ensure((size_t)(s->pgrid + s->cgrid + s->rgrid + s->tgrid + s->sgrid + s->lgrid + s->qgrid + s->egrid) *
                                 NST));
-        k_node_prep<<<s->pgrid, BLK, 0, s->stream>>>(a, s->bmask.p, s->bound.p, s->stat_part.p, s->ocnt.p,
-                                                     s->btot.p, s->pper, s->pscan.p, s->gcnt.p, (uint32_t)s->gcnt.n);
-        TRY(scan_desc(s, a));
+        if (!prepared)
+            k_node_prep<<<s->pgrid, BLK, 0, s->stream>>>(a, s->bmask.p, s->bound.p, s->stat_part.p, s->ocnt.p,
+                                                         s->btot.p, s->pper, s->pscan.p, s->gcnt.p, (uint32_t)s->gcnt.n);
+        TRY(scan_desc(s, a, prepared));
         if (batched) goto args;
         TRY(stream_wait(s));
         if (s->pin[PIN_BIGIN]) { s->pin[PIN_BIGIN] = 0; return PSIM_ENOMEM; }
@@ -2278,11 +2448,7 @@
 
 int route_group(psim_handle* h, Shard* s, bool dense, uint32_t m, bool fixed = false, bool exact = false) {
     const uint32_t n = s->n;
-    uint32_t wshift = n > (1u << 26) ? 13 : n > (1u << 22) ? 12 : 11;
-    if (const char* e = getenv("PSIM_ROUTE_WSHIFT")) {
-        const int v = atoi(e);
-        if (v >= (int)WSHIFT_MIN && v <= (int)WSHIFT_MAX) wshift = (uint32_t)v;
-    }
+    const uint32_t wshift = route_wshift(n);
     const uint32_t W = 1u << wshift, nb = (n + W - 1) >> wshift;
     const RouteIn in{s->outbox.p, s->okey.p, s->obase.p, s->ocnt.p, dense ? m : n, s->lo,
                      h->cfg.manager == PSIM_MANAGER_PLUGGABLE, dense ? s->recvh.p : nullptr,
@@ -2314,12 +2480,33 @@
         TRY(s->pairs.ensure((size_t)nb * capb));
         TRY(s->rank.ensure((size_t)nb * capb));
         static const uint32_t walk = getenv("PSIM_FILL_WALK") && atoi(getenv("PSIM_FILL_WALK")) ? 1u : 0u;
+        RoutePrep rp{};
+        if (s->prep_next) {
+            const psim_config& c = h->cfg;
+            uint32_t pshift = 0;
+            while ((1u << pshift) < s->pper) pshift++;
+            rp.round = s->prep_next - 1; rp.n_nodes = h->N; rp.lo = s->lo;
+            rp.shuffle_period = c.shuffle_period; rp.promotion_period = c.promotion_period;
+            rp.random_promotion = c.random_promotion; rp.plumtree = c.plumtree;
+            rp.lazy_tick_period = c.lazy_tick_period;
+            rp.xbot = c.manager == PSIM_MANAGER_XBOT; rp.xbot_period = c.xbot_period;
+            rp.pshift = pshift; rp.nranges = s->pgrid;
+            rp.flags = s->flags.p; rp.hdr = s->hdr.p; rp.pt_rt = s->pt_rt.p; rp.slots = s->slots.p;
+            rp.start = s->start.p; rp.packed = s->bound.p; rp.ocnt = s->ocnt.p; rp.tiles = s->pscan.p;
+            rp.btot = s->btot.p; rp.part = s->stat_part.p;
+        }
         k_bucket_fill<false><<<nblk, RB_STEP, lds_h, s->stream>>>(in, nsteps, nb, wshift, s->gcnt.p, capb, s->pairs.p,
                                                                   s->ctl.p, phase_end_mark(h, s), st, walk);
-        k_bucket_route<false><<<nb, RR_THREADS, lds_r, s->stream>>>(
-            n, wshift, h->rr_reg, nullptr, s->pairs.p, in.rec, nullptr, nullptr, s->rank.p, s->cb.p, s->bmask.p,
-            s->in_beg.p, s->ivals.p, s->tmp.p, s->inbox.p, s->pin_dev + PIN_M, s->rcap, s->ctl.p, s->gcnt.p, capb,
-            s->batch_round1, st, lcap);
+        if (s->prep_next)
+            k_bucket_route<false, true><<<nb, RR_THREADS, lds_r, s->stream>>>(
+                n, wshift, h->rr_reg, nullptr, s->pairs.p, in.rec, nullptr, nullptr, s->rank.p, s->cb.p, s->bmask.p,
+                s->in_beg.p, s->ivals.p, s->tmp.p, s->inbox.p, s->pin_dev + PIN_M, s->rcap, s->ctl.p, s->gcnt.p, capb,
+                s->batch_round1, st, lcap, rp);
+        else
+            k_bucket_route<false><<<nb, RR_THREADS, lds_r, s->stream>>>(
+                n, wshift, h->rr_reg, nullptr, s->pairs.p, in.rec, nullptr, nullptr, s->rank.p, s->cb.p, s->bmask.p,
+                s->in_beg.p, s->ivals.p, s->tmp.p, s->inbox.p, s->pin_dev + PIN_M, s->rcap, s->ctl.p, s->gcnt.p, capb,
+                s->batch_round1, st, lcap, rp);
         HIP_TRY(hipGetLastError());
         return PSIM_OK;
     }
@@ -2344,12 +2531,12 @@
         k_bucket_route<true><<<nb, RR_THREADS, lds_r, s->stream>>>(
             n, wshift, h->rr_reg, s->rbase.p, s->pairs.p, nullptr, in.wire, in.tails, s->rank.p, s->cb.p, s->bmask.p,
             s->in_beg.p, s->ivals.p, s->tmp.p, s->inbox.p, s->pin_dev + PIN_M, s->rcap, s->ctl.p, nullptr, 0u,
-            s->batch_round1, st, lcap);
+            s->batch_round1, st, lcap, RoutePrep{});
     else
         k_bucket_route<false><<<nb, RR_THREADS, lds_r, s->stream>>>(
             n, wshift, h->rr_reg, s->rbase.p, s->pairs.p, in.rec, nullptr, nullptr, s->rank.p, s->cb.p, s->bmask.p,
             s->in_beg.p, s->ivals.p, s->tmp.p, s->inbox.p, s->pin_dev + PIN_M, s->rcap, s->ctl.p, nullptr, 0u,
-            s->batch_round1, st, lcap);
+            s->batch_round1, st, lcap, RoutePrep{});
     HIP_TRY(hipGetLastError());
     return PSIM_OK;
 }
@@ -2772,14 +2959,22 @@
     s->tn = 0;
     s->desc_cap = batch_desc_cap(h, s);
     const auto t_enq = std::chrono::steady_clock::now();
+    uint32_t n_prepared = 0;
+    s->prepared = false;
     for (uint32_t j = 0; j < nb; j++) {
         s->stat_slot = j + 1;
         s->batch_round1 = (uint32_t)h->round + 1;
         RoundArgs a;
         const RoundCtl ctl = j == 0 ? ctl0 : RoundCtl{};
-        TRY(phase_events_prepare(h, s, ctl, a, j == 0, true));
+        TRY(phase_events_prepare(h, s, ctl, a, j == 0, true, false, s->prepared));
+        n_prepared += s->prepared;
         TRY(phase_consume(h, s, a));
+        const bool prep = j + 1 < nb && !ctl.crashes && prep_fused_handle(h, s) &&
+                          route_wshift(s->n) == WSHIFT_MIN && s->pper <= (1u << WSHIFT_MIN);
+        s->prep_next = prep ? (uint32_t)h->round + 2 : 0u;
+        s->prepared = prep;
         TRY(phase_route_local(h, s));
+        s->prep_next = 0;
         TRY(phase_stats(h, s, j == 0 ? crashed0 : none));
         if (j == 0 && bc0)
             k_origin<<<grid_for(h->pend_b_root.size()), BLK, 0, s->stream>>>(
@@ -2788,16 +2983,17 @@
         HIP_TRY(hipGetLastError());
         h->round++;
     }
-    s->stat_slot = 0; s->batch_round1 = 0; s->desc_cap = 0;
+    s->stat_slot = 0; s->batch_round1 = 0; s->desc_cap = 0; s->prepared = false;
     uint32_t cw[2] = {0, 0};
     HIP_TRY(hipMemcpyAsync(cw, s->ctl.p, sizeof cw, hipMemcpyDeviceToHost, s->stream));
     const auto t_wait = std::chrono::steady_clock::now();
     TRY(stream_wait(s));
     static const bool trace_batch = getenv("PSIM_TRACE_BATCH") != nullptr;
     if (trace_batch)
-        std::fprintf(stderr, "psim: batch of %u from round %llu: enqueue %.3f ms, wait %.3f ms\n", nb,
-                     (unsigned long long)r0, std::chrono::duration<double, std::milli>(t_wait - t_enq).count(),
-                     std::chrono::duration<double, std::milli>(std::chrono::steady_clock::now() - t_wait).count());
+        std::fprintf(stderr, "psim: batch of %u from round %llu: enqueue %.3f ms, wait %.3f ms, %u prepared in the route\n",
+                     nb, (unsigned long long)r0, std::chrono::duration<double, std::milli>(t_wait - t_enq).count(),
+                     std::chrono::duration<double, std::milli>(std::chrono::steady_clock::now() - t_wait).count(),
+                     n_prepared);
     if (s->pin[PIN_BIGIN]) {
         s->pin[PIN_BIGIN] = 0;
         HIP_TRY(hipMemsetAsync(s->ctl.p, 0, sizeof cw, s->stream));
diff --git a/profiles/round_kernels.py b/profiles/round_kernels.py
--- a/profiles/round_kernels.py
+++ b/profiles/round_kernels.py
@@ -9,7 +9,7 @@
 for r in rows:
     name = re.sub(r"\(.*", "", r["Kernel_Name"].replace("(anonymous namespace)::", "")).replace("void ", "").strip()
     d = (int(r["End_Timestamp"]) - int(r["Start_Timestamp"])) / 1e3
-    if "k_node_prep" in name:
+    if "k_node_prep" in name or ("k_desc" in name and (cur is None or any("k_desc" in k for k in cur))):
         cur = {"_start": int(r["Start_Timestamp"])}
         rounds.append(cur)
     if cur is not None:
```

After: 2.975 billion, median of 6. +3.2%, better.
